# PolarisRisingWar/rgb-experiment

Hardware: AMD Instinct MI355X
Metric: aggregated edges/sec (full-graph GCN d=128, reference epoch = train fwd+bwd+Adam + 2 eval fwd) (higher is better)
Workload: dtype f32

## Files before the change

include/rgbx_hip.h:

```cpp
#ifndef RGBX_HIP_H
#define RGBX_HIP_H

#include <stddef.h>
#include <stdint.h>

#ifdef __cplusplus
extern "C" {
#endif

#define RGBX_VERSION 501

#define RGBX_OK 0
#define RGBX_E_ARG (-1)
#define RGBX_E_RANGE (-2)
#define RGBX_E_ALIGN (-3)
#define RGBX_E_WS (-4)
#define RGBX_E_SHAPE (-5)

typedef void* rgbx_stream_t;

enum {
  RGBX_LOOPS_KEEP = 0,
  RGBX_LOOPS_ADD_REMAINING = 1,
  RGBX_LOOPS_REMOVE_ADD = 2
// ... 137 lines not shown
  int64_t N, K, Nout;
  const rgbx_row_split_t* split;
  const float* w_pos;
  float* z_pos_out;
  const uint8_t* col_sel;
} rgbx_fused_layer_t;

int rgbx_fused_layer_f32(const rgbx_fused_layer_t* layer, rgbx_stream_t stream);

int rgbx_blocked_to_rows_f32(const float* src, int64_t blk_cols, int64_t blk_stride, float* dst, int64_t ldd,
                             int64_t n, int64_t d, const float* bias, rgbx_stream_t stream);

int rgbx_appnp_f32(const int32_t* rowptr, const int32_t* col, const float* w, const float* h,
                   int64_t ldh, float* out, float* tmp, int64_t ldo, int64_t N, int64_t d, int K,
                   float alpha, const rgbx_row_split_t* split, rgbx_stream_t stream);


int rgbx_dagnn_gate_fwd_f32(const float* h0, int64_t ld0, const float* hops, int64_t hop_stride, int64_t ldh,
                            const float* s, const float* b, float* out, int64_t ldo, int64_t N, int64_t d, int K,
                            rgbx_stream_t stream);

int rgbx_dagnn_gate_bwd_workspace_bytes(int64_t d, size_t* bytes);
int rgbx_dagnn_gate_bwd_f32(const float* h0, int64_t ld0, const float* hops, int64_t hop_stride, int64_t ldh,
                            const float* s, const float* b, const float* gout, int64_t ldg, float* d0,
                            int64_t ldd0, float* dk, int64_t d_stride, int64_t ldd, float* g_s, float* g_b,
                            void* ws, size_t ws_bytes, int64_t N, int64_t d, int K, rgbx_stream_t stream);


int rgbx_gru_step_supported(int64_t C);
int rgbx_gru_step_f32(const int32_t* rowptr, const int32_t* col, const float* x, int64_t ldx, const float* wt,
                      const float* wt_root, const float* bias, float* out, int64_t ldo, float* z_out, int64_t ldz,
                      float* pre_out, int64_t ldp, int64_t N, int64_t C, const rgbx_row_split_t* split,
                      rgbx_stream_t stream);

int rgbx_gru_gate_fwd_f32(const float* pre, int64_t ldp, const float* x, int64_t ldx, float* out, int64_t ldo,
                          int64_t N, int64_t C, rgbx_stream_t stream);

int rgbx_gru_gate_bwd_f32(const float* pre, int64_t ldp, const float* x, int64_t ldx, const float* gout, int64_t ldg,
                          float* dpre, int64_t lddp, float* dx, int64_t lddx, int64_t N, int64_t C,
                          rgbx_stream_t stream);


int rgbx_gat_scores_f32(const float* hfeat, int64_t ldh, const float* att_src,
                        const float* att_dst, float* a_src, float* a_dst, int64_t n, int H, int C,
                        rgbx_stream_t stream);

int rgbx_gat_scores_bwd_scratch_floats(int64_t n, int H, int C, int64_t* count);

int rgbx_gat_scores_bwd_f32(const float* hfeat, int64_t ldh, const float* g_a_src, const float* g_a_dst,
                            int64_t n_dst, const float* att_src, const float* att_dst, float* g_hfeat,
                            int64_t ldgh, float* g_att_src, float* g_att_dst, float* scratch,
                            int64_t scratch_floats, int64_t n, int H, int C, rgbx_stream_t stream);

int rgbx_gat_aggregate_fwd_f32(const int32_t* rowptr, const int32_t* col, const float* hfeat,
                               int64_t ldh, const float* a_src, const float* att_src,
                               float* a_dst, const float* att_dst, const float* out_scale, const float* bias,
                               float* out, int64_t ldo, float* m, float* rden, float* out_pos, float* a_pos,
                               int64_t N, int H, int C, float slope, const rgbx_row_split_t* split,
                               rgbx_stream_t stream);

int rgbx_gat_edge_softmax_f32(const int32_t* rowptr, const int32_t* col, const float* a_src, const float* a_dst,
                              float slope, float* alpha, float* alpha_pos, float* m, float* rden, float* a_pos,
                              int64_t N, const rgbx_row_split_t* split, rgbx_stream_t stream);

int rgbx_gat_bwd_dst_f32(const int32_t* rowptr, const int32_t* col, const float* hfeat,
                         int64_t ldh, const float* a_src, const float* a_dst, const float* m,
                         const float* rden, const float* out, int64_t ldo, const float* gout,
                         int64_t ldg, float* nodeq, float* g_a_dst, int64_t N, int H, int C,
                         float slope, rgbx_stream_t stream);

int rgbx_gat_bwd_prep_f32(const float* a_dst, const float* m, const float* rden, const float* out,
                          int64_t ldo, const float* bias, const float* gout, int64_t ldg, float* nodeq,
                          const float* out_pos, const float* a_pos, float slope, float* g_a_dst,
                          int64_t N, int H, int C, rgbx_stream_t stream);

int rgbx_gat_bwd_src_f32(const int32_t* rowptr_t, const int32_t* col_t, const float* hfeat,
                         int64_t ldh, const float* a_src, const float* nodeq, const float* gout,
                         int64_t ldg, float* g_hfeat, int64_t ldgh, float* g_a_src, float* ds,
                         const float* att2, const float* g_a_dst, int64_t N, int H, int C, float slope,
                         const rgbx_row_split_t* split, rgbx_stream_t stream);



int rgbx_supergat_supported(int H, int C);

int rgbx_supergat_loss_records(int64_t N, const rgbx_row_split_t* split, int64_t* count);

int rgbx_supergat_aggregate_fwd_f32(const int32_t* rowptr, const int32_t* col, const float* hfeat, int64_t ldh,
                                    const float* att_l, const float* att_r, const float* bias, float* out, int64_t ldo,
                                    float* m, float* rden, int64_t N, int H, int C, float slope, const uint32_t* seed,
                                    float p_drop, float pos_ratio, float* loss_records, int64_t n_loss_records,
                                    double* pos_stats, const rgbx_row_split_t* split, rgbx_stream_t stream);

int rgbx_supergat_bwd_dst_f32(const int32_t* rowptr, const int32_t* col, const float* hfeat, int64_t ldh,
                              const float* att_l, const float* att_r, const float* m, const float* rden,
                              const float* out, int64_t ldo, const float* bias, const float* gout, int64_t ldg,
                              float* nodeq, float* g_hfeat, int64_t ldgh, float* g_ar, int64_t N, int H, int C,
                              float slope, const uint32_t* seed, float p_drop, float pos_ratio, const float* gl,
                              const rgbx_row_split_t* split, rgbx_stream_t stream);

int rgbx_supergat_bwd_src_f32(const int32_t* rowptr_t, const int32_t* col_t, const int32_t* t2f, const float* hfeat,
                              int64_t ldh, const float* att_l, const float* nodeq, const float* gout, int64_t ldg,
                              float* g_hfeat, int64_t ldgh, float* g_al, int64_t N, int H, int C, float slope,
                              const uint32_t* seed, float p_drop, float pos_ratio, const float* gl,
                              const rgbx_row_split_t* split, rgbx_stream_t stream);

int rgbx_supergat_sample_negatives(const uint64_t* keys, int64_t n_keys, int64_t N, const uint32_t* seed, int64_t n_neg,
                                   int redraws, int64_t* neg, uint8_t* valid, rgbx_stream_t stream);

int rgbx_supergat_neg_loss_fwd_f32(const float* hfeat, int64_t ldh, const int64_t* neg, const uint8_t* valid,
                                   int64_t n_neg, int H, int C, float* loss_records, int64_t n_loss_records,
                                   double* neg_stats, rgbx_stream_t stream);

int rgbx_supergat_neg_loss_bwd_f32(const float* hfeat, int64_t ldh, const int64_t* neg, const uint8_t* valid,
                                   int64_t n_neg, int H, int C, const float* gl, float* g_hfeat, int64_t ldgh,
                                   rgbx_stream_t stream);

int rgbx_supergat_draws_u8(const uint32_t* seed, int64_t nnz, int H, float p_drop, float pos_ratio, uint8_t* pos,
                           uint8_t* drop, rgbx_stream_t stream);



int rgbx_gatv2_supported(int H, int C);

int rgbx_gatv2_fwd_f32(const int32_t* rowptr, const int32_t* col, const float* xl, int64_t ldl, const float* xr,
                       int64_t ldr, const float* att, const float* bias, float* out, int64_t ldo, float* m, float* rden,
                       int64_t N, int H, int C, float slope, const uint32_t* seed, float p_drop,
                       const rgbx_row_split_t* split, rgbx_stream_t stream);

int rgbx_gatv2_att_partial_floats(int64_t N, int H, int C, const rgbx_row_split_t* split, int64_t* count);

int rgbx_gatv2_bwd_dst_f32(const int32_t* rowptr, const int32_t* col, const float* xl, int64_t ldl, const float* xr,
                           int64_t ldr, const float* att, const float* m, const float* rden, const float* out,
                           int64_t ldo, const float* bias, const float* gout, int64_t ldg, float* nodeq, float* g_xr,
                           int64_t ldgr, float* g_att, float* att_partial, int64_t n_att_partial, int64_t N, int H,
                           int C, float slope, const uint32_t* seed, float p_drop, const rgbx_row_split_t* split,
                           rgbx_stream_t stream);

int rgbx_gatv2_bwd_src_f32(const int32_t* rowptr_t, const int32_t* col_t, const int32_t* t2f, const float* xl,
                           int64_t ldl, const float* xr, int64_t ldr, const float* att, const float* nodeq,
                           const float* gout, int64_t ldg, float* g_xl, int64_t ldgl, int64_t N, int H, int C,
                           float slope, const uint32_t* seed, float p_drop, const rgbx_row_split_t* split,
                           rgbx_stream_t stream);

int rgbx_gatv2_draws_u8(const uint32_t* seed, int64_t nnz, int H, float p_drop, uint8_t* keep, rgbx_stream_t stream);


int rgbx_gemm_tn_workspace_bytes(int64_t K, int64_t M, int64_t N, size_t* bytes);

int rgbx_gemm_tn_f32(const float* A, int64_t lda, const float* B, int64_t ldb, float* C, int64_t ldc,
                     float* a_colsum, int64_t K, int64_t M, int64_t N, float alpha, void* workspace,
                     size_t workspace_bytes, rgbx_stream_t stream);


int rgbx_bn_scratch_doubles(int64_t N, int64_t d, int64_t* count);

int rgbx_bn_stats_f32(const float* x, int64_t ldx, int64_t N, int64_t d, double* sums, double* scratch,
                      int64_t scratch_doubles, rgbx_stream_t stream);

int rgbx_bn_finalize_f32(const double* packed, const float* weight, const float* bias, float eps, float momentum,
                         float* running_mean, float* running_var, float* mean, float* rstd, float* scale,
                         float* shift, int64_t d, rgbx_stream_t stream);

int rgbx_fold_bn_linear_f32(const float* W, int64_t ldw, const float* Wr, int64_t ldwr, const float* bias,
                            const float* bias2, const float* gamma, const float* beta, const float* running_mean,
                            const float* running_var, float eps, float* wt, float* wrt, float* b_out, int64_t Nout,
                            int64_t K, rgbx_stream_t stream);

int rgbx_bn_bwd_finalize_f32(const double* glob, const double* local, const double* count, const float* weight,
                             const float* rstd, float* ca, float* cb, float* ck, float* g_weight, float* g_bias,
                             int64_t d, rgbx_stream_t stream);

int rgbx_affine_cols_f32(const float* x, int64_t ldx, const float* scale, const float* shift, float* y,
                         int64_t ldy, int64_t N, int64_t d, rgbx_stream_t stream);

int rgbx_bn_bwd_reduce_f32(const float* gy, int64_t ldg, const float* x, int64_t ldx, const float* mean,
                           const float* rstd, int64_t N, int64_t d, double* sums, double* scratch,
                           int64_t scratch_doubles, rgbx_stream_t stream);

int rgbx_bn_bwd_apply_f32(const float* gy, int64_t ldg, const float* x, int64_t ldx, const float* mean,
                          const float* rstd, const float* ca, const float* cb, const float* ck, float* gx,
                          int64_t ldgx, int64_t N, int64_t d, rgbx_stream_t stream);


int rgbx_masked_nll_scratch_doubles(int64_t N, int want_accuracy, int64_t* count);

int rgbx_masked_nll_fwd_f32(const float* logp, int64_t ld, const int64_t* y, const uint8_t* mask,
                            int64_t N, int64_t C, double* stats, double* scratch,
                            int64_t scratch_doubles, int want_accuracy, rgbx_stream_t stream);

int rgbx_masked_nll_bwd_f32(const int64_t* y, const uint8_t* mask, int64_t N, int64_t C,
                            const float* scale, float* grad, int64_t ldg, rgbx_stream_t stream);

int rgbx_masked_ce_fwd_f32(const float* logits, int64_t ld, const int64_t* y, const uint8_t* mask, int64_t N,
                           int64_t C, double* stats, double* scratch, int64_t scratch_doubles,
                           rgbx_stream_t stream);

int rgbx_masked_ce_fwd_blocked_f32(const float* logits, int64_t blk_cols, int64_t blk_stride, const float* bias,
                                   const int64_t* y, const uint8_t* mask, int64_t N, int64_t C, double* stats,
                                   double* scratch, int64_t scratch_doubles, rgbx_stream_t stream);

int rgbx_masked_ce_bwd_f32(const float* logits, int64_t ld, const int64_t* y, const uint8_t* mask, int64_t N,
                           int64_t C, const float* scale, float* grad, int64_t ldg, rgbx_stream_t stream);


int rgbx_coalesce_workspace_bytes(int64_t E, int64_t N, int mirror, size_t* bytes);
int rgbx_coalesce_keys_i64(const int64_t* row, const int64_t* col, int64_t E, int64_t N, int mirror,
                           uint64_t* keys_out, uint64_t* counts, void* workspace, size_t workspace_bytes,
                           rgbx_stream_t stream);
int rgbx_split_edge_keys_i64(const uint64_t* keys, const uint64_t* counts, int64_t cap, int64_t N, int64_t* out_row,
                             int64_t* out_col, rgbx_stream_t stream);

int rgbx_py_random_shuffle_i64(int64_t seed, int64_t n, int64_t* perm);


int rgbx_gather_rows_f32(const float* src, int64_t lds, const int32_t* idx, int64_t n, int64_t d,
                         float* dst, int64_t ldd, rgbx_stream_t stream);

int rgbx_scatter_add_rows_f32(const float* src, int64_t lds, const int32_t* idx, int64_t n,
                              int64_t d, float* dst, int64_t ldd, rgbx_stream_t stream);

int rgbx_paced_copy_f32(const float* src, float* dst, int64_t n, int workgroups, int nontemporal, rgbx_stream_t stream);



int rgbx_faconv_supported(int64_t C);

int rgbx_faconv_scores_f32(const float* x, int64_t ldx, const float* att_l, const float* att_r, float* alr, int64_t N,
                           int64_t C, rgbx_stream_t stream);

int rgbx_faconv_fwd_f32(const int32_t* rowptr, const int32_t* col, const float* w, const float* x, int64_t ldx,
                        const float* alr, const float* x0, int64_t ldx0, float eps, float* out, int64_t ldo, int64_t N,
                        int64_t C, const uint32_t* seed, float p_drop, const rgbx_row_split_t* split,
                        rgbx_stream_t stream);

int rgbx_faconv_bwd_dst_f32(const int32_t* rowptr, const int32_t* col, const float* w, const float* x, int64_t ldx,
                            const float* alr, const float* gout, int64_t ldg, float* g_alr, int64_t N, int64_t C,
                            const uint32_t* seed, float p_drop, const rgbx_row_split_t* split, rgbx_stream_t stream);

int rgbx_faconv_bwd_src_f32(const int32_t* rowptr_t, const int32_t* col_t, const float* w_t, const int32_t* t2f,
                            const float* x, int64_t ldx, const float* alr, const float* gout, int64_t ldg,
                            const float* att_l, const float* att_r, float* g_alr, float* g_x, int64_t ldgx, int64_t N,
                            int64_t C, const uint32_t* seed, float p_drop, const rgbx_row_split_t* split,
                            rgbx_stream_t stream);

int rgbx_faconv_edge_coef_f32(const int32_t* rowptr, const int32_t* col, const float* w, const int32_t* slot,
                              const float* alr, int transposed, int64_t N, const uint32_t* seed, float p_drop,
                              float* coef, float* q, rgbx_stream_t stream);

int rgbx_faconv_edge_dot_f32(const int32_t* rowptr, const int32_t* col, const float* q, const float* a, int64_t lda,
                             const float* b, int64_t ldb, float* out, int64_t out_stride, int64_t N, int64_t C,
                             rgbx_stream_t stream);

int rgbx_faconv_draws_u8(const uint32_t* seed, int64_t nnz, float p_drop, uint8_t* keep, rgbx_stream_t stream);

#ifdef __cplusplus
}
#endif
#endif
```

rgb_experiment_amd/_lib.py:

```python
import ctypes
import os

import torch

_HERE = os.path.dirname(os.path.abspath(__file__))
LIB_PATH = os.path.join(_HERE, "csrc", "librgbx_hip.so")

_P = ctypes.c_void_p
_I64 = ctypes.c_int64
_I = ctypes.c_int
_F = ctypes.c_float

class RowSplit(ctypes.Structure):
    _fields_ = [("threshold", ctypes.c_int32), ("n_chunks", ctypes.c_int32), ("n_long", ctypes.c_int32),
                ("chunk_begin", ctypes.c_void_p), ("chunk_end", ctypes.c_void_p), ("chunk_row", ctypes.c_void_p),
                ("long_row", ctypes.c_void_p),
                ("long_chunk_ptr", ctypes.c_void_p), ("partial", ctypes.c_void_p)]


class CeEpilogue(ctypes.Structure):
    _fields_ = [("y", ctypes.c_void_p), ("mask", ctypes.c_void_p), ("grad_scale", ctypes.c_void_p),
                ("stats", ctypes.c_void_p), ("scratch", ctypes.c_void_p), ("mask_groups", ctypes.c_int32),
                ("rows", ctypes.c_void_p), ("n_rows", ctypes.c_int64), ("skip_unselected", ctypes.c_int32)]


class SpmmEpilogue(ctypes.Structure):
    _fields_ = [("ce", ctypes.c_void_p), ("n_classes", ctypes.c_int64), ("out_colsums", ctypes.c_void_p),
                ("stats_ws", ctypes.c_void_p), ("stats_ws_bytes", ctypes.c_size_t)]


class FusedLayer(ctypes.Structure):
    _fields_ = [("rowptr", _P), ("col", _P), ("w", _P), ("rs", _P), ("x", _P), ("ldx", _I64),
                ("x_blk_cols", _I64), ("x_blk_stride", _I64), ("wt", _P), ("x_root", _P), ("ldr", _I64),
                ("xr_blk_cols", _I64), ("xr_blk_stride", _I64), ("wt_root", _P), ("bias", _P), ("out", _P),
                ("ldo", _I64), ("out_blk", _P), ("ob_cols", _I64), ("ob_stride", _I64), ("z_out", _P), ("ldz", _I64),
                ("pre_scale", _P), ("pre_shift", _P), ("pre_rowsum", _P), ("out_colsums", _P), ("stats_ws", _P),
                ("stats_ws_bytes", ctypes.c_size_t), ("ce", _P), ("N", _I64), ("K", _I64), ("Nout", _I64),
                ("split", _P), ("w_pos", _P), ("z_pos_out", _P), ("col_sel", _P)]


SIGNATURES = {
    "rgbx_csr_workspace_bytes": [_I64, _I64, ctypes.POINTER(ctypes.c_size_t)],
    "rgbx_csr_build": [_P, _P, _I64, _I64, _I, _P, _P, _P, _P, ctypes.c_size_t, _P],
    "rgbx_deg_inv_sqrt_f32": [_P, _I64, _P, _P],
    "rgbx_gcn_norm_f32": [_P, _P, _I64, _P, _P, _P],
    "rgbx_inv_degree_f32": [_P, _I64, _P, _P],
    "rgbx_loop_weights_f32": [_P, _P, _P, _I64, _I64, _I, _F, _P, _P, _P],
    "rgbx_edge_slot_weights_f32": [_P, _I64, _P, _I64, _P, _P, _P],
    "rgbx_weighted_deg_inv_sqrt_f32": [_P, _P, _I64, _P, _P],
    "rgbx_gcn_norm_weighted_f32": [_P, _P, _P, _I64, _P, _P, _P],
    "rgbx_edge_dot_supported": [_I64],
    "rgbx_edge_dot_f32": [_P, _P, _P, _I64, _P, _I64, _P, _I64, _I64, _P, _P],
    "rgbx_gcn_norm_bwd_f32": [_P, _P, _P, _P, _P, _P, _P, _P, _P, _P, _I64, _I64, _P, _P, _P],
    "rgbx_spmm_csr_f32": [_P, _P, _P, _P, _P, _I64, _P, _I64, _P, _P, _I64, _I64, _I64, _F, _F, _P, _P],
    "rgbx_spmm_csr_extremum_supported": [_I64],
    "rgbx_spmm_csr_extremum_f32": [_P, _P, _P, _I64, _P, _I64, _P, _I64, _I64, _I, _P, _P],
    "rgbx_extremum_bwd_f32": [_P, _P, _P, _P, _I64, _P, _P, _I64, _I64, _I64, _P, _P],
    "rgbx_spmm_csr_epilogue_supported": [_I64],
    "rgbx_spmm_csr_epilogue_f32": [_P, _P, _P, _P, _P, _I64, _P, _I64, _P, _P, _I64, _I64, _I64, _F, _F, _P, _P, _P],
    "rgbx_spmm_csr_short_rows_supported": [_I64],
    "rgbx_spmm_csr_short_rows_f32": [_P, _P, _P, _P, _I64, _P, _P, _I64, _I64, _I64, _P],
    "rgbx_spmm_linear_supported": [_I64, _I64, _I],
    "rgbx_spmm_linear_stats_workspace_bytes": [_I64, _I64, ctypes.POINTER(ctypes.c_size_t)],
    "rgbx_spmm_linear_f32": [_P, _P, _P, _P, _P, _I64, _P, _P, _I64, _P, _P, _P, _I64, _P, _I64, _P, _P, _P, _P, _P,
                             ctypes.c_size_t, _P, _I64, _I64, _I64, _P, _P],
    "rgbx_fused_layer_f32": [_P, _P],
    "rgbx_blocked_to_rows_f32": [_P, _I64, _I64, _P, _I64, _I64, _I64, _P, _P],
    "rgbx_appnp_f32": [_P, _P, _P, _P, _I64, _P, _P, _I64, _I64, _I64, _I, _F, _P, _P],
    "rgbx_dagnn_gate_fwd_f32": [_P, _I64, _P, _I64, _I64, _P, _P, _P, _I64, _I64, _I64, _I, _P],
    "rgbx_dagnn_gate_bwd_workspace_bytes": [_I64, ctypes.POINTER(ctypes.c_size_t)],
    "rgbx_dagnn_gate_bwd_f32": [_P, _I64, _P, _I64, _I64, _P, _P, _P, _I64, _P, _I64, _P, _I64, _I64, _P, _P, _P,
                                ctypes.c_size_t, _I64, _I64, _I, _P],
    "rgbx_gru_step_supported": [_I64],
    "rgbx_gru_step_f32": [_P, _P, _P, _I64, _P, _P, _P, _P, _I64, _P, _I64, _P, _I64, _I64, _I64, _P, _P],
    "rgbx_gru_gate_fwd_f32": [_P, _I64, _P, _I64, _P, _I64, _I64, _I64, _P],
    "rgbx_gru_gate_bwd_f32": [_P, _I64, _P, _I64, _P, _I64, _P, _I64, _P, _I64, _I64, _I64, _P],
    "rgbx_gat_scores_f32": [_P, _I64, _P, _P, _P, _P, _I64, _I, _I, _P],
    "rgbx_gat_scores_bwd_scratch_floats": [_I64, _I, _I, ctypes.POINTER(ctypes.c_int64)],
    "rgbx_gat_scores_bwd_f32": [_P, _I64, _P, _P, _I64, _P, _P, _P, _I64, _P, _P, _P, _I64, _I64, _I, _I, _P],
    "rgbx_gat_aggregate_fwd_f32": [_P, _P, _P, _I64, _P, _P, _P, _P, _P, _P, _P, _I64, _P, _P, _P, _P, _I64, _I, _I, _F, _P,
                                   _P],
    "rgbx_gat_edge_softmax_f32": [_P, _P, _P, _P, _F, _P, _P, _P, _P, _P, _I64, _P, _P],
    "rgbx_gat_bwd_dst_f32": [_P, _P, _P, _I64, _P, _P, _P, _P, _P, _I64, _P, _I64, _P, _P, _I64, _I, _I,
                             _F, _P],
    "rgbx_gat_bwd_prep_f32": [_P, _P, _P, _P, _I64, _P, _P, _I64, _P, _P, _P, _F, _P, _I64, _I, _I, _P],
    "rgbx_gat_bwd_src_f32": [_P, _P, _P, _I64, _P, _P, _P, _I64, _P, _I64, _P, _P, _P, _P, _I64, _I, _I, _F, _P, _P],
    "rgbx_supergat_supported": [_I, _I],
    "rgbx_supergat_loss_records": [_I64, _P, ctypes.POINTER(ctypes.c_int64)],
    "rgbx_supergat_aggregate_fwd_f32": [_P, _P, _P, _I64, _P, _P, _P, _P, _I64, _P, _P, _I64, _I, _I, _F, _P, _F, _F, _P,
                                        _I64, _P, _P, _P],
    "rgbx_supergat_bwd_dst_f32": [_P, _P, _P, _I64, _P, _P, _P, _P, _P, _I64, _P, _P, _I64, _P, _P, _I64, _P, _I64, _I, _I,
                                  _F, _P, _F, _F, _P, _P, _P],
    "rgbx_supergat_bwd_src_f32": [_P, _P, _P, _P, _I64, _P, _P, _P, _I64, _P, _I64, _P, _I64, _I, _I, _F, _P, _F, _F, _P,
                                  _P, _P],
    "rgbx_supergat_sample_negatives": [_P, _I64, _I64, _P, _I64, _I, _P, _P, _P],
    "rgbx_supergat_neg_loss_fwd_f32": [_P, _I64, _P, _P, _I64, _I, _I, _P, _I64, _P, _P],
    "rgbx_supergat_neg_loss_bwd_f32": [_P, _I64, _P, _P, _I64, _I, _I, _P, _P, _I64, _P],
    "rgbx_supergat_draws_u8": [_P, _I64, _I, _F, _F, _P, _P, _P],
    "rgbx_gatv2_supported": [_I, _I],
    "rgbx_gatv2_fwd_f32": [_P, _P, _P, _I64, _P, _I64, _P, _P, _P, _I64, _P, _P, _I64, _I, _I, _F, _P, _F, _P, _P],
    "rgbx_gatv2_att_partial_floats": [_I64, _I, _I, _P, ctypes.POINTER(ctypes.c_int64)],
    "rgbx_gatv2_bwd_dst_f32": [_P, _P, _P, _I64, _P, _I64, _P, _P, _P, _P, _I64, _P, _P, _I64, _P, _P, _I64, _P, _P, _I64,
                               _I64, _I, _I, _F, _P, _F, _P, _P],
    "rgbx_gatv2_bwd_src_f32": [_P, _P, _P, _P, _I64, _P, _I64, _P, _P, _P, _I64, _P, _I64, _I64, _I, _I, _F, _P, _F, _P,
                               _P],
    "rgbx_gatv2_draws_u8": [_P, _I64, _I, _F, _P, _P],
    "rgbx_gemm_tn_workspace_bytes": [_I64, _I64, _I64, ctypes.POINTER(ctypes.c_size_t)],
    "rgbx_gemm_tn_f32": [_P, _I64, _P, _I64, _P, _I64, _P, _I64, _I64, _I64, _F, _P, ctypes.c_size_t, _P],
    "rgbx_bn_scratch_doubles": [_I64, _I64, ctypes.POINTER(ctypes.c_int64)],
    "rgbx_bn_stats_f32": [_P, _I64, _I64, _I64, _P, _P, _I64, _P],
    "rgbx_bn_finalize_f32": [_P, _P, _P, _F, _F, _P, _P, _P, _P, _P, _P, _I64, _P],
    "rgbx_fold_bn_linear_f32": [_P, _I64, _P, _I64, _P, _P, _P, _P, _P, _P, _F, _P, _P, _P, _I64, _I64, _P],
    "rgbx_bn_bwd_finalize_f32": [_P, _P, _P, _P, _P, _P, _P, _P, _P, _P, _I64, _P],
    "rgbx_affine_cols_f32": [_P, _I64, _P, _P, _P, _I64, _I64, _I64, _P],
    "rgbx_bn_bwd_reduce_f32": [_P, _I64, _P, _I64, _P, _P, _I64, _I64, _P, _P, _I64, _P],
    "rgbx_bn_bwd_apply_f32": [_P, _I64, _P, _I64, _P, _P, _P, _P, _P, _P, _I64, _I64, _I64, _P],
    "rgbx_masked_nll_scratch_doubles": [_I64, _I, ctypes.POINTER(ctypes.c_int64)],
    "rgbx_masked_nll_fwd_f32": [_P, _I64, _P, _P, _I64, _I64, _P, _P, _I64, _I, _P],
    "rgbx_masked_ce_fwd_f32": [_P, _I64, _P, _P, _I64, _I64, _P, _P, _I64, _P],
    "rgbx_masked_ce_fwd_blocked_f32": [_P, _I64, _I64, _P, _P, _P, _I64, _I64, _P, _P, _I64, _P],
    "rgbx_masked_ce_bwd_f32": [_P, _I64, _P, _P, _I64, _I64, _P, _P, _I64, _P],
    "rgbx_masked_nll_bwd_f32": [_P, _P, _I64, _I64, _P, _P, _I64, _P],
    "rgbx_coalesce_workspace_bytes": [_I64, _I64, _I, ctypes.POINTER(ctypes.c_size_t)],
    "rgbx_coalesce_keys_i64": [_P, _P, _I64, _I64, _I, _P, _P, _P, ctypes.c_size_t, _P],
    "rgbx_split_edge_keys_i64": [_P, _P, _I64, _I64, _P, _P, _P],
    "rgbx_gather_rows_f32": [_P, _I64, _P, _I64, _I64, _P, _I64, _P],
    "rgbx_scatter_add_rows_f32": [_P, _I64, _P, _I64, _I64, _P, _I64, _P],
    "rgbx_paced_copy_f32": [_P, _P, _I64, _I, _I, _P],
    "rgbx_py_random_shuffle_i64": [_I64, _I64, _P],
    "rgbx_faconv_supported": [_I64],
    "rgbx_faconv_scores_f32": [_P, _I64, _P, _P, _P, _I64, _I64, _P],
    "rgbx_faconv_fwd_f32": [_P, _P, _P, _P, _I64, _P, _P, _I64, _F, _P, _I64, _I64, _I64, _P, _F, _P, _P],
    "rgbx_faconv_bwd_dst_f32": [_P, _P, _P, _P, _I64, _P, _P, _I64, _P, _I64, _I64, _P, _F, _P, _P],
    "rgbx_faconv_bwd_src_f32": [_P, _P, _P, _P, _P, _I64, _P, _P, _I64, _P, _P, _P, _P, _I64, _I64, _I64, _P, _F, _P,
                                _P],
    "rgbx_faconv_edge_coef_f32": [_P, _P, _P, _P, _P, _I, _I64, _P, _F, _P, _P, _P],
    "rgbx_faconv_edge_dot_f32": [_P, _P, _P, _P, _I64, _P, _I64, _P, _I64, _I64, _I64, _P],
    "rgbx_faconv_draws_u8": [_P, _I64, _F, _P, _P],
}
EXPORTS = ["rgbx_version", "rgbx_last_error_string"] + list(SIGNATURES)

_lib = None


def bind(path, strict=True):
    lib = ctypes.CDLL(path)
    lib.rgbx_version.restype = _I
    lib.rgbx_version.argtypes = []
    lib.rgbx_last_error_string.restype = ctypes.c_char_p
    lib.rgbx_last_error_string.argtypes = []
    for name, argtypes in SIGNATURES.items():
        if not strict and not hasattr(lib, name):
            continue
        fn = getattr(lib, name)
        fn.restype = _I
        fn.argtypes = argtypes
    return lib


def load():
    global _lib
    if _lib is not None:
        return _lib
    if not os.path.exists(LIB_PATH):
        raise RuntimeError(
            f"rgb_experiment_amd: {LIB_PATH} is not built — run `python -c 'import __graft_entry__ as g; "
            "g.build()'` (or `make -C rgb_experiment_amd/csrc`). There is no CPU fallback.")
    _lib = bind(LIB_PATH)
    return _lib


def use(lib):
    global _lib
    _lib = lib


def check(rc, what):
    if rc != 0:
        msg = load().rgbx_last_error_string().decode(errors="replace")
        kind = "argument error" if rc < 0 else "hipError"
        raise RuntimeError(f"{what} failed ({kind} {rc}): {msg}")


def require_device(*tensors):
    for t in tensors:
        if t is not None and not t.is_cuda:
            raise RuntimeError(
                "rgb_experiment_amd: the message-passing path runs in HIP kernels on an MI355X device; "
                f"got a tensor on '{t.device}'. There is no CPU fallback (oracle/ is test-only).")


def stream_ptr():
    return torch.cuda.current_stream().cuda_stream


def ptr(t):
    return 0 if t is None else t.data_ptr()


def mat(t, name="tensor"):
    if t.dtype != torch.float32 or t.dim() != 2:
        raise RuntimeError(f"{name}: expected a 2-D float32 tensor, got {t.dtype} {tuple(t.shape)}")
    if t.size(1) > 1 and t.stride(1) != 1:
        raise RuntimeError(f"{name}: rows must be contiguous (stride {t.stride()})")
    ld = t.stride(0) if t.size(0) > 1 else max(t.size(1), 1)
    return t.data_ptr(), ld
```

rgb_experiment_amd/csrc/bn.hip:

```cpp
#include "rgbx_common.h"

namespace rgbx {
namespace {

constexpr int kMaxBlocks = 1024;

struct ColMap {
  int cv;
  int rg;
};

__host__ __device__ inline ColMap col_map(int d, int vec) {
  int cv = (d + vec - 1) / vec;
  if (cv > 256) cv = 256;
  ColMap m{cv, 256 / cv};
  return m;
}

template <int VEC, bool BWD>
__global__ void __launch_bounds__(256)
col_reduce_kernel(const float* __restrict__ a, int64_t lda, const float* __restrict__ b, int64_t ldb,
                  const float* __restrict__ mean, const float* __restrict__ rstd, int64_t N, int d,
                  double* __restrict__ part) {
  extern __shared__ double sh[];
  const ColMap M = col_map(d, VEC);
  const int tid = threadIdx.x;
  const int cvi = tid % M.cv, rgi = tid / M.cv;
  const bool thread_ok = rgi < M.rg;
  const int stride_c = M.cv * VEC;
  for (int cbase = 0; cbase < d; cbase += stride_c) {
    const int c = cbase + cvi * VEC;
    const bool active = thread_ok && c < d;
    double s0[VEC], s1[VEC];
    float mu[VEC], rs[VEC];
#pragma unroll
    for (int i = 0; i < VEC; ++i) { s0[i] = s1[i] = 0.0; mu[i] = 0.f; rs[i] = 1.f; }
    if (BWD && active) {
      load_vec<VEC>(mu, mean + c);
      load_vec<VEC>(rs, rstd + c);
    }
    if (active) {
      for (int64_t r = (int64_t)blockIdx.x * M.rg + rgi; r < N; r += (int64_t)gridDim.x * M.rg) {
        float va[VEC];
        load_vec<VEC>(va, a + r * lda + c);
        if constexpr (BWD) {
          float vb[VEC];
          load_vec<VEC>(vb, b + r * ldb + c);
#pragma unroll
          for (int i = 0; i < VEC; ++i) {
            s0[i] += (double)va[i];
            s1[i] += (double)(va[i] * ((vb[i] - mu[i]) * rs[i]));
          }
        } else {
#pragma unroll
          for (int i = 0; i < VEC; ++i) {
            s0[i] += (double)va[i];
            s1[i] += (double)va[i] * (double)va[i];
          }
        }
      }
    }
    __syncthreads();
    if (thread_ok) {
#pragma unroll
      for (int i = 0; i < VEC; ++i) {
        sh[(rgi * 2 + 0) * stride_c + cvi * VEC + i] = s0[i];
        sh[(rgi * 2 + 1) * stride_c + cvi * VEC + i] = s1[i];
      }
    }
    __syncthreads();
    if (rgi == 0 && active) {
#pragma unroll
      for (int i = 0; i < VEC; ++i) {
        if (c + i < d) {
          double t0 = 0.0, t1 = 0.0;
          for (int g = 0; g < M.rg; ++g) {
            t0 += sh[(g * 2 + 0) * stride_c + cvi * VEC + i];
            t1 += sh[(g * 2 + 1) * stride_c + cvi * VEC + i];
          }
          part[((int64_t)blockIdx.x * 2 + 0) * d + c + i] = t0;
          part[((int64_t)blockIdx.x * 2 + 1) * d + c + i] = t1;
        }
      }
    }
  }
}

__global__ void __launch_bounds__(256)
col_finish_kernel(const double* __restrict__ part, int n_blocks, int d, double* __restrict__ sums) {
  __shared__ double sh[32][8];
  const int j = threadIdx.x & 7, q = threadIdx.x >> 3;
  const int c = blockIdx.x * 8 + j;
  double s = 0.0;
  if (c < 2 * d) {
    const int which = c / d, col = c % d;
    for (int b = q; b < n_blocks; b += 32) s += part[((int64_t)b * 2 + which) * d + col];
  }
  sh[q][j] = s;
  __syncthreads();
  if (q == 0 && c < 2 * d) {
    double t = 0.0;
#pragma unroll
    for (int k = 0; k < 32; ++k) t += sh[k][j];
    sums[c] = t;
  }
}

template <int VEC>
__global__ void __launch_bounds__(256)
affine_kernel(const float* __restrict__ x, int64_t ldx, const float* __restrict__ scale,
              const float* __restrict__ shift, float* __restrict__ y, int64_t ldy, int64_t N, int d) {
  const int per_row = (d + VEC - 1) / VEC;
  const int64_t total = N * per_row;
  for (int64_t idx = (int64_t)blockIdx.x * blockDim.x + threadIdx.x; idx < total;
       idx += (int64_t)gridDim.x * blockDim.x) {
    const int64_t r = idx / per_row;
    const int c = (int)(idx % per_row) * VEC;
    float v[VEC], sc[VEC], sf[VEC];
    load_vec<VEC>(v, x + r * ldx + c);
    load_vec<VEC>(sc, scale + c);
    load_vec<VEC>(sf, shift + c);
#pragma unroll
    for (int i = 0; i < VEC; ++i) v[i] = fmaf(v[i], sc[i], sf[i]);
    store_vec<VEC>(y + r * ldy + c, v);
  }
}

template <int VEC>
__global__ void __launch_bounds__(256)
bn_bwd_apply_kernel(const float* __restrict__ gy, int64_t ldg, const float* __restrict__ x, int64_t ldx,
                    const float* __restrict__ mean, const float* __restrict__ rstd, const float* __restrict__ ca,
                    const float* __restrict__ cb, const float* __restrict__ ck, float* __restrict__ gx,
                    int64_t ldgx, int64_t N, int d) {
  const int per_row = (d + VEC - 1) / VEC;
  const int64_t total = N * per_row;
  for (int64_t idx = (int64_t)blockIdx.x * blockDim.x + threadIdx.x; idx < total;
       idx += (int64_t)gridDim.x * blockDim.x) {
    const int64_t r = idx / per_row;
    const int c = (int)(idx % per_row) * VEC;
    float g[VEC], v[VEC], mu[VEC], rs[VEC], a[VEC], b[VEC], k[VEC];
    load_vec<VEC>(g, gy + r * ldg + c);
    load_vec<VEC>(v, x + r * ldx + c);
    load_vec<VEC>(mu, mean + c);
    load_vec<VEC>(rs, rstd + c);
    load_vec<VEC>(a, ca + c);
    load_vec<VEC>(b, cb + c);
    load_vec<VEC>(k, ck + c);
#pragma unroll
    for (int i = 0; i < VEC; ++i) g[i] = (g[i] - a[i] - (v[i] - mu[i]) * rs[i] * b[i]) * k[i];
    store_vec<VEC>(gx + r * ldgx + c, g);
  }
}

int reduce_grid(int64_t N, int d, int vec) {
  const ColMap M = col_map(d, vec);
  int64_t b = cdiv(N, (int64_t)M.rg * 16);
  if (b > kMaxBlocks) b = kMaxBlocks;
  return (int)(b < 1 ? 1 : b);
}

bool vec4_ok(int64_t d, std::initializer_list<const void*> ptrs, std::initializer_list<int64_t> lds) {
  bool ok = d % 4 == 0;
  for (const void* p : ptrs) ok = ok && aligned16(p);
  for (int64_t ld : lds) ok = ok && ld % 4 == 0;
  return ok;
}

template <bool BWD>
int run_reduce(const float* a, int64_t lda, const float* b, int64_t ldb, const float* mean, const float* rstd,
               int64_t N, int64_t d, double* sums, double* scratch, int64_t scratch_doubles, hipStream_t s,
               const char* name) {
  if (N < 0 || d <= 0 || !sums) return fail(RGBX_E_ARG, "%s: bad argument", name);
  if (d >= INT32_MAX) return fail(RGBX_E_RANGE, "%s: d exceeds int32", name);
  if (N == 0) {
    RGBX_HIP(hipMemsetAsync(sums, 0, 2 * d * sizeof(double), s));
    return RGBX_OK;
  }
  if (!a || lda < d || (BWD && (!b || ldb < d || !mean || !rstd)) || !scratch)
    return fail(RGBX_E_ARG, "%s: null pointer or leading dimension < d", name);
  const bool v4 = BWD ? vec4_ok(d, {a, b, mean, rstd}, {lda, ldb}) : vec4_ok(d, {a}, {lda});
  const int vec = v4 ? 4 : 1;
  const int grid = reduce_grid(N, (int)d, vec);
  if (scratch_doubles < (int64_t)grid * 2 * d)
    return fail(RGBX_E_WS, "%s: scratch %lld < %lld doubles", name, (long long)scratch_doubles,
                (long long)grid * 2 * d);
  const ColMap M = col_map((int)d, vec);
  const size_t lds = (size_t)M.rg * 2 * M.cv * vec * sizeof(double);
  if (v4)
    col_reduce_kernel<4, BWD><<<grid, 256, lds, s>>>(a, lda, b, ldb, mean, rstd, N, (int)d, scratch);
  else
    col_reduce_kernel<1, BWD><<<grid, 256, lds, s>>>(a, lda, b, ldb, mean, rstd, N, (int)d, scratch);
  RGBX_CHECK_LAUNCH(name);
  col_finish_kernel<<<(int)cdiv(2 * d, 8), 256, 0, s>>>(scratch, grid, (int)d, sums);
  RGBX_CHECK_LAUNCH("col_finish_kernel");
  return RGBX_OK;
}

__global__ void __launch_bounds__(256)
bn_finalize_kernel(const double* __restrict__ packed, const float* __restrict__ weight,
                   const float* __restrict__ bias, float eps, float momentum, float* __restrict__ running_mean,
                   float* __restrict__ running_var, float* __restrict__ mean, float* __restrict__ rstd,
                   float* __restrict__ scale, float* __restrict__ shift, int d) {
  const int c = blockIdx.x * blockDim.x + threadIdx.x;
  if (c >= d) return;
  const double n = packed[2 * d];
  const double m64 = packed[c] / n;
  double v64 = packed[d + c] / n - m64 * m64;
  v64 = v64 > 0.0 ? v64 : 0.0;
  const float m = (float)m64, var = (float)v64;
  const float r = 1.0f / sqrtf(var + eps);
  const float sc = weight[c] * r;
  mean[c] = m;
  rstd[c] = r;
  scale[c] = sc;
  shift[c] = bias[c] - m * sc;
  if (running_mean) {
    const double nm1 = n > 1.0 ? n - 1.0 : 1.0;
    const float unbiased = var * (float)(n / nm1);
    running_mean[c] = running_mean[c] * (1.0f - momentum) + momentum * m;
    running_var[c] = running_var[c] * (1.0f - momentum) + momentum * unbiased;
  }
}

__global__ void __launch_bounds__(256)
bn_bwd_finalize_kernel(const double* __restrict__ glob, const double* __restrict__ local,
                       const double* __restrict__ count, const float* __restrict__ weight,
                       const float* __restrict__ rstd, float* __restrict__ ca, float* __restrict__ cb,
                       float* __restrict__ ck, float* __restrict__ g_weight, float* __restrict__ g_bias, int d) {
  const int c = blockIdx.x * blockDim.x + threadIdx.x;
  if (c >= d) return;
  const double n = *count;
  ca[c] = (float)(glob[c] / n);
  cb[c] = (float)(glob[d + c] / n);
  ck[c] = weight[c] * rstd[c];
  g_bias[c] = (float)local[c];
  g_weight[c] = (float)local[d + c];
}

__global__ void __launch_bounds__(256)
fold_bn_linear_kernel(const float* __restrict__ W, int64_t ldw, const float* __restrict__ Wr, int64_t ldwr,
                      const float* __restrict__ bias, const float* __restrict__ bias2,
                      const float* __restrict__ gamma, const float* __restrict__ beta,
                      const float* __restrict__ rmean, const float* __restrict__ rvar, float eps,
                      float* __restrict__ wt, float* __restrict__ wrt, float* __restrict__ b_out, int Nout, int K) {
  __shared__ float tile[2][32][33];
  __shared__ float sc[32];
  const int n0 = blockIdx.x * 32, k0 = blockIdx.y * 32;
  const int tx = threadIdx.x & 31, ty = threadIdx.x >> 5;
  if (threadIdx.x < 32) {
    const int n = n0 + threadIdx.x;
    float s = 1.f, t = 0.f;
    if (n < Nout && gamma) {
      s = gamma[n] * (1.0f / sqrtf(rvar[n] + eps));
      t = beta[n] - rmean[n] * s;
    }
    sc[threadIdx.x] = s;
    if (n < Nout && b_out && blockIdx.y == 0) {
      float b = bias ? bias[n] : 0.f;
      if (bias2) b += bias2[n];
      b_out[n] = b * s + t;
    }
  }
  for (int r = ty; r < 32; r += 8) {
    const int n = n0 + r, k = k0 + tx;
    const bool ok = n < Nout && k < K;
    tile[0][r][tx] = ok ? W[(int64_t)n * ldw + k] : 0.f;
    if (Wr) tile[1][r][tx] = ok ? Wr[(int64_t)n * ldwr + k] : 0.f;
  }
  __syncthreads();
  for (int r = ty; r < 32; r += 8) {
    const int k = k0 + r, n = n0 + tx;
    if (k < K && n < Nout) {
      wt[(int64_t)k * Nout + n] = tile[0][tx][r] * sc[tx];
      if (Wr) wrt[(int64_t)k * Nout + n] = tile[1][tx][r] * sc[tx];
    }
  }
}

int elt_grid(int64_t total) {
  int64_t b = cdiv(total, 256);
  return (int)(b < kMaxGrid ? (b < 1 ? 1 : b) : kMaxGrid);
}

}
}

using namespace rgbx;

extern "C" int rgbx_fold_bn_linear_f32(const float* W, int64_t ldw, const float* Wr, int64_t ldwr, const float* bias,
                                       const float* bias2, const float* gamma, const float* beta,
                                       const float* running_mean, const float* running_var, float eps, float* wt,
                                       float* wrt, float* b_out, int64_t Nout, int64_t K, rgbx_stream_t stream) {
  if (Nout <= 0 || K <= 0) return fail(RGBX_E_ARG, "fold_bn_linear: bad size");
  if (!W || !wt || (Wr && !wrt)) return fail(RGBX_E_ARG, "fold_bn_linear: null pointer");
  const bool bn = gamma || beta || running_mean || running_var;
  if (bn && !(gamma && beta && running_mean && running_var))
    return fail(RGBX_E_ARG, "fold_bn_linear: gamma, beta, running_mean and running_var go together");
  if (ldw < K || (Wr && ldwr < K)) return fail(RGBX_E_ARG, "fold_bn_linear: leading dimension too small");
  if (Nout >= INT32_MAX || K >= INT32_MAX) return fail(RGBX_E_RANGE, "fold_bn_linear: size exceeds int32");
  dim3 grid((unsigned)cdiv(Nout, 32), (unsigned)cdiv(K, 32));
  fold_bn_linear_kernel<<<grid, 256, 0, (hipStream_t)stream>>>(W, ldw, Wr, ldwr, bias, bias2, gamma, beta, running_mean,
                                                            running_var, eps, wt, wrt, b_out, (int)Nout, (int)K);
// ... 80 lines not shown
```

rgb_experiment_amd/csrc/gemm.hip:

```cpp
#include "rgbx_common.h"

namespace rgbx {
namespace {

constexpr int BM = 128, BN = 128, KT = 32;
using f32x16 = __attribute__((ext_vector_type(16))) float;

template <int W>
__device__ __forceinline__ void stage_tile(float* __restrict__ lds, const float* __restrict__ src,
                                           int64_t ld, int64_t k0, int64_t k_end, int c0, int ncols) {
  const int tid = threadIdx.x;
#pragma unroll 4
  for (int p = 0; p < KT * W / 256; ++p) {
    const int idx = p * 256 + tid;
    const int r = idx / W, c = idx % W;
    const int64_t k = k0 + r;
    lds[r * W + c] = (k < k_end && c0 + c < ncols) ? src[k * ld + c0 + c] : 0.f;
  }
}

template <int W>
__device__ __forceinline__ void fetch_tile(float4 (&regs)[KT * (W / 4) / 256], const float* __restrict__ src, int64_t ld,
                                           int64_t k0, int64_t k_end, int c0, int ncols) {
#pragma unroll
  for (int p = 0; p < KT * (W / 4) / 256; ++p) {
    const int idx = p * 256 + threadIdx.x;
    const int r = idx / (W / 4), c = (idx % (W / 4)) * 4;
    const int64_t k = k0 + r;
    regs[p] = make_float4(0.f, 0.f, 0.f, 0.f);
    if (k < k_end && c0 + c < ncols) regs[p] = *reinterpret_cast<const float4*>(src + k * ld + c0 + c);
  }
}

template <int W>
__device__ __forceinline__ void put_tile(float* __restrict__ lds, const float4 (&regs)[KT * (W / 4) / 256]) {
#pragma unroll
  for (int p = 0; p < KT * (W / 4) / 256; ++p) {
    const int idx = p * 256 + threadIdx.x;
    const int r = idx / (W / 4), c = (idx % (W / 4)) * 4;
    *reinterpret_cast<float4*>(lds + r * W + c) = regs[p];
  }
}

template <bool VEC4, int MT>
__global__ void __launch_bounds__(256)
gemm_tn_partial_kernel(const float* __restrict__ A, int64_t lda, const float* __restrict__ B, int64_t ldb,
                       float* __restrict__ part, float* __restrict__ colpart, int64_t K, int M, int N,
                       int64_t slab) {
  constexpr int MI = MT / 64;
  __shared__ float lds[KT * (MT + 128)];
  float* la = lds;
  float* lb = lds + KT * MT;
  const int split = blockIdx.x;
  const int m0 = blockIdx.y * MT, n0 = blockIdx.z * BN;
  const int64_t k_begin = (int64_t)split * slab;
  const int64_t k_end = k_begin + slab < K ? k_begin + slab : K;
  const int wave = threadIdx.x >> 6, lane = threadIdx.x & 63;
  const int wm = (wave >> 1) * (MT / 2), wn = (wave & 1) * 64;
  const int kr = lane >> 5, cc = lane & 31;

  f32x16 acc[MI][2];
#pragma unroll
  for (int i = 0; i < MI; ++i)
#pragma unroll
    for (int j = 0; j < 2; ++j)
#pragma unroll
      for (int r = 0; r < 16; ++r) acc[i][j][r] = 0.f;

  const bool sums = colpart != nullptr && blockIdx.z == 0 && threadIdx.x < MT;
  float csum = 0.f;
  auto consume = [&]() {
    if (sums) {
#pragma unroll 8
      for (int r = 0; r < KT; ++r) csum += la[r * MT + threadIdx.x];
    }
#pragma unroll 4
    for (int kk = 0; kk < KT; kk += 2) {
      float a[MI];
#pragma unroll
      for (int i = 0; i < MI; ++i) a[i] = la[(kk + kr) * MT + wm + i * 32 + cc];
      const float b0 = lb[(kk + kr) * 128 + wn + cc];
      const float b1 = lb[(kk + kr) * 128 + wn + 32 + cc];
#pragma unroll
      for (int i = 0; i < MI; ++i) {
        acc[i][0] = __builtin_amdgcn_mfma_f32_32x32x2f32(a[i], b0, acc[i][0], 0, 0, 0);
        acc[i][1] = __builtin_amdgcn_mfma_f32_32x32x2f32(a[i], b1, acc[i][1], 0, 0, 0);
      }
    }
  };
  if constexpr (VEC4) {
    float4 ra[KT * (MT / 4) / 256], rb[KT * 32 / 256];
    fetch_tile<MT>(ra, A, lda, k_begin, k_end, m0, M);
    fetch_tile<128>(rb, B, ldb, k_begin, k_end, n0, N);
    for (int64_t k0 = k_begin; k0 < k_end; k0 += KT) {
      __syncthreads();
      put_tile<MT>(la, ra);
      put_tile<128>(lb, rb);
      __syncthreads();
      if (k0 + KT < k_end) {
        fetch_tile<MT>(ra, A, lda, k0 + KT, k_end, m0, M);
        fetch_tile<128>(rb, B, ldb, k0 + KT, k_end, n0, N);
      }
      consume();
    }
  } else {
    for (int64_t k0 = k_begin; k0 < k_end; k0 += KT) {
      __syncthreads();
      stage_tile<MT>(la, A, lda, k0, k_end, m0, M);
      stage_tile<128>(lb, B, ldb, k0, k_end, n0, N);
      __syncthreads();
      consume();
    }
  }

  if (sums && m0 + (int)threadIdx.x < M) colpart[(int64_t)split * M + m0 + threadIdx.x] = csum;
  float* out = part + (int64_t)split * M * N;
#pragma unroll
  for (int i = 0; i < MI; ++i)
#pragma unroll
    for (int j = 0; j < 2; ++j)
#pragma unroll
      for (int r = 0; r < 16; ++r) {
        const int m = m0 + wm + i * 32 + (r & 3) + 8 * (r >> 2) + 4 * kr;
        const int n = n0 + wn + j * 32 + cc;
        if (m < M && n < N) out[(int64_t)m * N + n] = acc[i][j][r];
      }
}

__global__ void __launch_bounds__(256)
gemm_tn_reduce_kernel(const float* __restrict__ part, int S, int64_t MN, float* __restrict__ C, int N,
                      int64_t ldc, float alpha) {
  __shared__ float sh[8][32];
  const int j = threadIdx.x & 31, q = threadIdx.x >> 5;
  for (int64_t base = (int64_t)blockIdx.x * 32; base < MN; base += (int64_t)gridDim.x * 32) {
    const int64_t i = base + j;
    float s = 0.f;
    if (i < MN)
      for (int p = q; p < S; p += 8) s += part[(int64_t)p * MN + i];
    __syncthreads();
    sh[q][j] = s;
    __syncthreads();
    if (q == 0 && i < MN) {
      float t = 0.f;
#pragma unroll
      for (int k = 0; k < 8; ++k) t += sh[k][j];
      C[(i / N) * ldc + (i % N)] = alpha * t;
    }
  }
}

int tile_rows(int M) { return M <= 64 ? 64 : BM; }

int choose_splits(int64_t K, int M, int N) {
  const int64_t tiles = cdiv(M, tile_rows(M)) * cdiv(N, BN);
  int64_t s = cdiv(tile_rows(M) == 64 ? 1024 : 768, tiles);
  const int64_t max_s = cdiv(K, 16 * KT);
  if (s > max_s) s = max_s;
  if (s < 1) s = 1;
  return (int)s;
}

}
}

using namespace rgbx;

extern "C" int rgbx_gemm_tn_workspace_bytes(int64_t K, int64_t M, int64_t N, size_t* bytes) {
  if (!bytes || K < 0 || M < 0 || N < 0) return fail(RGBX_E_ARG, "gemm_tn_workspace_bytes: bad argument");
  if (M >= INT32_MAX || N >= INT32_MAX) return fail(RGBX_E_RANGE, "gemm_tn: M or N exceeds int32");
  *bytes = (size_t)choose_splits(K, (int)M, (int)N) * ((size_t)M * (size_t)N + (size_t)M) * sizeof(float);
  return RGBX_OK;
}

extern "C" int rgbx_gemm_tn_f32(const float* A, int64_t lda, const float* B, int64_t ldb, float* C,
                                int64_t ldc, float* a_colsum, int64_t K, int64_t M, int64_t N, float alpha,
                                void* workspace, size_t workspace_bytes, rgbx_stream_t stream) {
  if (K < 0 || M < 0 || N < 0) return fail(RGBX_E_ARG, "gemm_tn: negative size");
  if (M == 0 || N == 0) return RGBX_OK;
  if (!C || (K > 0 && (!A || !B))) return fail(RGBX_E_ARG, "gemm_tn: null pointer");
  if (M >= INT32_MAX || N >= INT32_MAX) return fail(RGBX_E_RANGE, "gemm_tn: M or N exceeds int32");
  if (lda < M || ldb < N || ldc < N) return fail(RGBX_E_ARG, "gemm_tn: leading dimension too small");
  size_t need = 0;
  if (int rc = rgbx_gemm_tn_workspace_bytes(K, M, N, &need)) return rc;
  if (!workspace || workspace_bytes < need)
    return fail(RGBX_E_WS, "gemm_tn: workspace %zu < %zu bytes", workspace_bytes, need);
  hipStream_t s = (hipStream_t)stream;
  const int S = choose_splits(K, (int)M, (int)N);
  const int64_t slab = cdiv(cdiv(K > 0 ? K : 1, S), KT) * KT;
  float* part = static_cast<float*>(workspace);
  float* colpart = a_colsum ? part + (size_t)S * M * N : nullptr;
  const int mt = tile_rows((int)M);
  dim3 grid(S, (unsigned)cdiv(M, mt), (unsigned)cdiv(N, BN));
  const bool v4 = aligned16(A) && aligned16(B) && lda % 4 == 0 && ldb % 4 == 0;
#define RGBX_GEMM_TN(V4, MT) \
  gemm_tn_partial_kernel<V4, MT><<<grid, 256, 0, s>>>(A, lda, B, ldb, part, colpart, K, (int)M, (int)N, slab)
  if (v4) { if (mt == 64) RGBX_GEMM_TN(true, 64); else RGBX_GEMM_TN(true, 128); }
  else { if (mt == 64) RGBX_GEMM_TN(false, 64); else RGBX_GEMM_TN(false, 128); }
#undef RGBX_GEMM_TN
  RGBX_CHECK_LAUNCH("gemm_tn_partial_kernel");
  const int64_t MN = M * N;
  int64_t rb = cdiv(MN, 32);
  if (rb > kMaxGrid) rb = kMaxGrid;
  gemm_tn_reduce_kernel<<<(int)rb, 256, 0, s>>>(part, S, MN, C, (int)N, ldc, alpha);
  RGBX_CHECK_LAUNCH("gemm_tn_reduce_kernel");
  if (a_colsum) {
    gemm_tn_reduce_kernel<<<(int)cdiv(M, 32), 256, 0, s>>>(colpart, S, M, a_colsum, (int)M, M, 1.0f);
    RGBX_CHECK_LAUNCH("gemm_tn_reduce_kernel");
  }
  return RGBX_OK;
}
```

rgb_experiment_amd/csrc/rgbx_common.h:

```cpp
#pragma once
#include <cstring>
#include <hip/hip_runtime.h>

#include <algorithm>
#include <cstdarg>
#include <cstdint>
#include <cstdio>
#include <initializer_list>

#include "../../include/rgbx_hip.h"

namespace rgbx {

constexpr int kWave = 64;

char* err_buf();

inline int fail(int code, const char* fmt, ...) {
  va_list ap;
  va_start(ap, fmt);
  vsnprintf(err_buf(), 256, fmt, ap);
  va_end(ap);
  return code;
}

inline int hip_fail(hipError_t e, const char* what) {
  snprintf(err_buf(), 256, "%s: %s", what, hipGetErrorString(e));
  return (int)e;
}

#define RGBX_CHECK_LAUNCH(what)                               \
  do {                                                        \
    hipError_t e_ = hipGetLastError();                        \
    if (e_ != hipSuccess) return ::rgbx::hip_fail(e_, what);  \
  } while (0)

#define RGBX_HIP(call)                                         \
  do {                                                         \
    hipError_t e_ = (call);                                    \
    if (e_ != hipSuccess) return ::rgbx::hip_fail(e_, #call);  \
  } while (0)

inline bool aligned16(const void* p) { return (reinterpret_cast<uintptr_t>(p) & 15u) == 0; }

inline int64_t cdiv(int64_t a, int64_t b) { return (a + b - 1) / b; }

template <int VEC> struct VecT;
template <> struct VecT<4> { using type = float4; };
template <> struct VecT<2> { using type = float2; };
template <> struct VecT<1> { using type = float; };

template <int VEC>
__device__ __forceinline__ void load_vec(float (&v)[VEC], const float* p) {
  using V = typename VecT<VEC>::type;
  const V t = *reinterpret_cast<const V*>(p);
  if constexpr (VEC == 4) { v[0] = t.x; v[1] = t.y; v[2] = t.z; v[3] = t.w; }
  else if constexpr (VEC == 2) { v[0] = t.x; v[1] = t.y; }
  else { v[0] = t; }
}

template <int VEC>
__device__ __forceinline__ void store_vec(float* p, const float (&v)[VEC]) {
  using V = typename VecT<VEC>::type;
  V t;
  if constexpr (VEC == 4) { t.x = v[0]; t.y = v[1]; t.z = v[2]; t.w = v[3]; }
  else if constexpr (VEC == 2) { t.x = v[0]; t.y = v[1]; }
  else { t = v[0]; }
  *reinterpret_cast<V*>(p) = t;
}

constexpr int kMaxGrid = 256 * 8 * 4;

}
```

rgb_experiment_amd/models/_stack.py:

```python
import torch
import torch.nn as nn
import torch.nn.functional as F

from ..nn import BatchNorm1d


class ModelOutput(dict):

    _LAZY = ("out", "x")

    def __init__(self, logits):
        super().__init__(emb=logits)

    def _log_probs(self):
        out = F.log_softmax(dict.__getitem__(self, "emb"), dim=1)
        dict.__setitem__(self, "out", out)
        dict.__setitem__(self, "x", out)
        return out

    def __missing__(self, key):
        if key in self._LAZY:
            return self._log_probs()
        raise KeyError(key)

    def get(self, key, default=None):
        if key in self._LAZY and not dict.__contains__(self, key):
            return self._log_probs()
        return dict.get(self, key, default)

    def __contains__(self, key):
        return key in self._LAZY or dict.__contains__(self, key)

    def keys(self):
        return ["out", "emb", "x"]

    def __iter__(self):
        return iter(self.keys())

    def __len__(self):
        return 3

    def values(self):
        return [self[k] for k in self.keys()]

    def items(self):
        return [(k, self[k]) for k in self.keys()]

    def copy(self):
        return dict(self.items())

    def pop(self, key, *default):
        if key in self._LAZY and not dict.__contains__(self, key):
            self._log_probs()
        return dict.pop(self, key, *default)

    def __eq__(self, other):
        return dict(self.items()) == other

    __hash__ = None

    def __repr__(self):
        return repr(dict(self.items()))


def model_output(logits):
    return ModelOutput(logits)


class ConvStack(nn.Module):

    def __init__(self, num_layers, dropout_rate, widths, make_conv, bn_width):
        super().__init__()
        if num_layers < 2:
            raise ValueError("num_layers must be at least 2")
        self.num_layers = num_layers
        self.dropout_rate = dropout_rate
        self.convs = nn.ModuleList(make_conv(i, widths[i], widths[i + 1]) for i in range(num_layers))
        self.bns = nn.ModuleList(BatchNorm1d(bn_width) for _ in range(num_layers - 1))

    def forward(self, x, edge_index, edge_weight=None):
        return model_output(self._run(x, edge_index, edge_weight=edge_weight))

    def masked_ce(self, x, edge_index, y, mask, edge_weight=None):
        return self._run(x, edge_index, ce=(y, mask), edge_weight=edge_weight)

    def masked_ce_pair(self, x, edge_index, y, mask_a, mask_b, edge_weight=None):
        return self._run(x, edge_index, ce=(y, (mask_a, mask_b)), edge_weight=edge_weight)[1]

    def _run(self, x, edge_index, ce=None, edge_weight=None):
        from .. import ops
        last = self.num_layers - 1
        ew = {}
        if edge_weight is not None:
            if any(type(c).__name__ != "GCNConv" for c in self.convs):
                raise ValueError(f"{type(self).__name__}: edge_weight is taken by stacks of GCNConv only")
            ew["edge_weight"] = edge_weight
        learned = edge_weight is not None and edge_weight.requires_grad and torch.is_grad_enabled()
        pending = None
        if self.training and torch.is_grad_enabled():
            self._train_forwards = getattr(self, "_train_forwards", 0) + 1
        folded = self._eval_operands() if (not torch.is_grad_enabled() and not self.training and x.is_cuda) else None
        agg0 = (self._input_aggregate(x, edge_index, edge_weight)
                if getattr(self, "cache_input_aggregate", False) and not learned else None)
        if folded is not None and agg0 is None and getattr(self, "collapse_eval", True):
            out = self._run_collapsed(x, edge_index, ce, edge_weight)
            if out is not None:
                return out
        for i, conv in enumerate(self.convs):
            bn = self.bns[i] if i < last else None
            if i == 0 and agg0 is not None and i < last:
                if folded is not None and folded[0] is not None:
                    x = conv.forward_from_aggregate(agg0, x, folded=folded[0])
                    continue
                if torch.is_grad_enabled() or bn is None or bn.training:
                    want = (bn is not None and bn.training and torch.is_grad_enabled()
                            and hasattr(bn, "begin_training_step"))
                    x, pending = conv.forward_from_aggregate(agg0, x, want_colsums=want), bn
                    continue
            if folded is not None and pending is None and folded[i] is not None:
                res = conv.forward_folded(x, edge_index, folded[i], ce=ce if i == last else None, **ew)
                if res is not None:
                    x = res
                    continue
            extra = dict(ew)
            if (bn is not None and bn.training and torch.is_grad_enabled() and getattr(conv, "emits_colsums", False)
                    and hasattr(bn, "begin_training_step")):
                extra["want_colsums"] = True
            if (i == last and ce is not None and getattr(conv, "accepts_ce", False)
                    and (not isinstance(ce[1], (tuple, list)) or getattr(conv, "accepts_ce_pair", False))):
                extra["ce"] = ce
            if pending is not None:
                sums = getattr(x, ops.COLSUMS, None)
                after = getattr(conv, "forward_after_bn", None)
                if after is not None:
                    x, pending = after(x, edge_index, pending, colsums=sums, **extra), bn
                    continue
                x, pending = (pending(x, colsums=sums) if sums is not None else pending(x)), None
            affine = None
            if bn is not None and getattr(conv, "folds_post_affine", False) and not torch.is_grad_enabled():
                fold = getattr(bn, "eval_affine", None)
                affine = fold() if fold is not None else None
            if affine is not None:
                x = conv(x, edge_index, post_affine=affine, **ew)
            else:
                x, pending = conv(x, edge_index, **extra), bn
        if ce is not None and not isinstance(x, tuple):
            x = ops.ce_from_logits(x, ce[0], ce[1])
        return x


def _layer_maps(conv):
    from ..graph import LOOPS_ADD_REMAINING, LOOPS_KEEP, LOOPS_REMOVE_ADD
    name = type(conv).__name__
    if getattr(conv, "aggr", "mean") != "mean":
        return None
    if name == "GCNConv":
        return conv.lin.weight, None, conv.bias, "gcn", LOOPS_ADD_REMAINING
    if name == "MySAGEConv" and conv.add_self_loops:
        return conv.lin_l.weight, conv.lin_r.weight, conv.lin_l.bias + conv.lin_r.bias, "mean", LOOPS_REMOVE_ADD
    if name == "SAGEConv":
        return conv.lin_l.weight, conv.lin_r.weight, conv.lin_l.bias, "mean", LOOPS_KEEP
    return None


def _collapsed_operands(self):
    from .. import ops
    tensors = list(self.parameters()) + list(self.buffers())
    key = (getattr(self, "_train_forwards", 0), ops.weights_epoch()) + tuple((t._version, t.data_ptr()) for t in tensors)
    cached = getattr(self, "_collapsed", None)
    if cached is not None and cached[0] == key:
        return cached[1]
    out = None
    convs, last = list(self.convs), self.num_layers - 1
    maps = [_layer_maps(c) for c in convs]
    C = getattr(convs[-1], "out_channels", 0)
    Cp = (C + 3) // 4 * 4
    if (all(m is not None for m in maps) and len({(m[3], m[4]) for m in maps}) == 1 and 0 < Cp <= 256
            and all(c.out_channels > Cp for c in convs[:-1])):
        affines = [getattr(self.bns[i], "eval_affine", lambda: None)() for i in range(last)]
        if all(a is not None for a in affines):
            with torch.no_grad():
                Q, d = None, None
                for l, (wl, wr, b, _, _) in enumerate(maps):
                    scale, shift = affines[l] if l < last else (None, None)
                    ml = wl.t() if scale is None else wl.t() * scale[None, :]
                    mr = None if wr is None else (wr.t() if scale is None else wr.t() * scale[None, :])
                    if Q is None:
                        Q, d = [mr, ml], [None, None]
                    else:
                        nq, nd = [None] * (len(Q) + 1), [None] * (len(Q) + 1)
                        for k in range(len(Q)):
                            for src, m, dst in ((Q, mr, k), (Q, ml, k + 1)):
                                if src[k] is not None and m is not None:
                                    nq[dst] = src[k] @ m if nq[dst] is None else nq[dst] + src[k] @ m
                            for m, dst in ((mr, k), (ml, k + 1)):
                                if d[k] is not None and m is not None:
                                    nd[dst] = d[k] @ m if nd[dst] is None else nd[dst] + d[k] @ m
                        Q, d = nq, nd
                    const = b if scale is None else b * scale + shift
                    d[0] = const if d[0] is None else d[0] + const
                pad = torch.nn.functional.pad
                have = [k for k, q in enumerate(Q) if q is not None]
                weight = torch.cat([pad(Q[k].t(), (0, 0, 0, Cp - C)) for k in have], dim=0).contiguous()
                shifts = [None if v is None else pad(v.detach(), (0, Cp - C)).contiguous() for v in d]
                out = (weight, have, shifts, C, Cp, maps[0][3], maps[0][4])
    self._collapsed = (key, out)
    return out


def _run_collapsed(self, x, edge_index, ce, edge_weight=None):
    from .. import ops
    from ..graph import get_graph
    operands = self._collapsed_operands()
    if operands is None:
        return None
    weight, have, shifts, C, Cp, kind, loops_mode = operands
    graph = get_graph(edge_index, x.size(0), loops_mode, edge_weight)
    if getattr(graph, "is_distributed", False) or not ops.rows_epilogue_ok(graph, Cp, x, None if ce is None else ce[0]):
        return None
    z = ops.linear(x, weight)
    block = {k: z[:, j * Cp:(j + 1) * Cp] for j, k in enumerate(have)}
    w, rs = ops._kind_weights(graph, kind)
    top = len(shifts) - 1
    u = block[top]
    for k in range(top - 1, 0, -1):
        u = ops.spmm_raw(graph.fwd, w, rs, u, y=block.get(k), a=1.0, b=1.0, bias=shifts[k], kind=f"{kind}_fwd")
    if ce is None:
        return ops.spmm_raw(graph.fwd, w, rs, u, y=block.get(0), a=1.0, b=1.0, bias=shifts[0], kind=f"{kind}_fwd")[:, :C]
    labels, mask = ce
    _, stats = ops.spmm_epilogue_raw(graph.fwd, w, rs, u, y=block.get(0), a=1.0, b=1.0, bias=shifts[0],
                                     ce=(labels, mask, None), n_classes=C, kind=f"{kind}_fwd")
    return None, stats


ConvStack._collapsed_operands = _collapsed_operands
ConvStack._run_collapsed = _run_collapsed


def _eval_operands(self):
    tensors = list(self.parameters()) + list(self.buffers())
    from .. import ops
    key = (getattr(self, "_train_forwards", 0), ops.weights_epoch()) + tuple((t._version, t.data_ptr()) for t in tensors)
    cached = getattr(self, "_folded_eval", None)
    if cached is None or cached[0] != key:
        last = self.num_layers - 1
        out = []
        for i, conv in enumerate(self.convs):
            bn = self.bns[i] if i < last else None
            make = getattr(conv, "eval_operands", None)
            ok = make is not None and (bn is None or (hasattr(bn, "eval_affine") and bn.affine and bn.track_running_stats))
            out.append(make(bn) if ok else None)
        cached = (key, out)
        self._folded_eval = cached
    return cached[1]


ConvStack._eval_operands = _eval_operands


def _input_aggregate(self, x, edge_index, edge_weight=None):
    if x.requires_grad or not x.is_cuda:
        return None
    key = (x.data_ptr(), x._version, tuple(x.shape), edge_index.data_ptr(), edge_index._version, tuple(edge_index.shape))
    if edge_weight is not None:
        key += (edge_weight.data_ptr(), edge_weight._version, tuple(edge_weight.shape))
    cached = getattr(self, "_agg0", None)
    if cached is None or cached[0] != key:
        make = getattr(self.convs[0], "aggregate_input", None)
        args = (x, edge_index) if edge_weight is None else (x, edge_index, edge_weight)
        cached = (key, make(*args) if make is not None else None, x, edge_index, edge_weight)
        self._agg0 = cached
    return cached[1]


ConvStack._input_aggregate = _input_aggregate


def _weighted_call(fn, fwd):
    import inspect
    return set(fwd) == {"x", "edge_index", "edge_weight"} and "edge_weight" in inspect.signature(fn).parameters


def masked_ce_pair(model, fwd, y, mask_a, mask_b):
    from .. import ops
    fn = getattr(model, "masked_ce_pair", None)
    if fn is not None and set(fwd) == {"x", "edge_index"} and fwd["x"].is_cuda:
        return fn(fwd["x"], fwd["edge_index"], y, mask_a, mask_b)
    if fn is not None and fwd["x"].is_cuda and _weighted_call(fn, fwd):
        return fn(fwd["x"], fwd["edge_index"], y, mask_a, mask_b, edge_weight=fwd["edge_weight"])
    emb = model(**fwd)["emb"]
    return torch.stack([ops.masked_ce_accuracy(emb, y, mask_a), ops.masked_ce_accuracy(emb, y, mask_b)])


def masked_ce(model, fwd, y, mask):
    from .. import ops
    fn = getattr(model, "masked_ce", None)
    if fn is not None and set(fwd) == {"x", "edge_index"} and fwd["x"].is_cuda:
        return fn(fwd["x"], fwd["edge_index"], y, mask)
    if fn is not None and fwd["x"].is_cuda and _weighted_call(fn, fwd):
        return fn(fwd["x"], fwd["edge_index"], y, mask, edge_weight=fwd["edge_weight"])
    return ops.ce_from_logits(model(**fwd)["emb"], y, mask)
# ... 1 lines not shown
```

rgb_experiment_amd/nn/batchnorm.py:

```python
import ctypes

import torch
import torch.nn as nn

from .. import _lib


def _scratch(n, d, device):
    cnt = ctypes.c_int64(0)
    _lib.check(_lib.load().rgbx_bn_scratch_doubles(n, d, ctypes.byref(cnt)), "rgbx_bn_scratch_doubles")
    return torch.empty(cnt.value, dtype=torch.float64, device=device), cnt.value


def column_sums(x):
    if not x.is_cuda:
        xd = x.double()
        return torch.stack([xd.sum(0), (xd * xd).sum(0)])
    px, ldx = _lib.mat(x, "x")
    n, d = x.shape
    sums = torch.empty((2, d), dtype=torch.float64, device=x.device)
    scratch, cnt = _scratch(n, d, x.device)
    _lib.check(_lib.load().rgbx_bn_stats_f32(px, ldx, n, d, _lib.ptr(sums), _lib.ptr(scratch), cnt, _lib.stream_ptr()),
               "rgbx_bn_stats_f32")
    return sums


def affine_cols(x, scale, shift):
    if not x.is_cuda:
        return x * scale + shift
    px, ldx = _lib.mat(x, "x")
    y = torch.empty((x.size(0), x.size(1)), dtype=torch.float32, device=x.device)
    _lib.check(_lib.load().rgbx_affine_cols_f32(px, ldx, _lib.ptr(scale), _lib.ptr(shift), _lib.ptr(y), y.stride(0),
                                                x.size(0), x.size(1), _lib.stream_ptr()), "rgbx_affine_cols_f32")
    return y


def bwd_sums(gy, x, mean, rstd):
    if not gy.is_cuda:
        xhat = (x - mean) * rstd
        return torch.stack([gy.double().sum(0), (gy * xhat).double().sum(0)])
    pg, ldg = _lib.mat(gy, "gy")
    px, ldx = _lib.mat(x, "x")
    n, d = x.shape
    sums = torch.empty((2, d), dtype=torch.float64, device=x.device)
    scratch, cnt = _scratch(n, d, x.device)
    _lib.check(_lib.load().rgbx_bn_bwd_reduce_f32(pg, ldg, px, ldx, _lib.ptr(mean), _lib.ptr(rstd), n, d, _lib.ptr(sums),
                                                  _lib.ptr(scratch), cnt, _lib.stream_ptr()), "rgbx_bn_bwd_reduce_f32")
    return sums


def bwd_apply(gy, x, mean, rstd, ca, cb, ck):
    if not gy.is_cuda:
        return (gy - ca - (x - mean) * rstd * cb) * ck
    pg, ldg = _lib.mat(gy, "gy")
    px, ldx = _lib.mat(x, "x")
    gx = torch.empty((x.size(0), x.size(1)), dtype=torch.float32, device=x.device)
    _lib.check(_lib.load().rgbx_bn_bwd_apply_f32(pg, ldg, px, ldx, _lib.ptr(mean), _lib.ptr(rstd), _lib.ptr(ca),
                                                 _lib.ptr(cb), _lib.ptr(ck), _lib.ptr(gx), gx.stride(0), x.size(0),
                                                 x.size(1), _lib.stream_ptr()), "rgbx_bn_bwd_apply_f32")
    return gx


class _BNTrain(torch.autograd.Function):

    @staticmethod
    def forward(ctx, x, weight, bias, eps, reduce, running, colsums=None):
        x = x if x.stride(-1) == 1 else x.contiguous()
        mean, rstd, scale, shift, n = train_statistics(x, weight, bias, eps, reduce, running, colsums)
        y = affine_cols(x, scale.contiguous(), shift.contiguous())
        ctx.save_for_backward(x, weight, mean, rstd, n)
        ctx.reduce = reduce
        return y

    @staticmethod
    def backward(ctx, gy):
        x, weight, mean, rstd, n = ctx.saved_tensors
        gx, gw, gb = train_backward(gy, x, weight, mean, rstd, n, ctx.reduce)
        return gx, gw, gb, None, None, None, None


def pack_statistics(x, colsums=None):
    d = x.size(1)
    count = torch.full((1,), float(x.size(0)), dtype=torch.float64, device=x.device)
    sums = colsums if colsums is not None and tuple(colsums.shape) == (2, d) else column_sums(x)
    return torch.cat([sums.reshape(-1), count])


def train_statistics(x, weight, bias, eps, reduce, running, colsums=None, packed=None):
    d = x.size(1)
    if packed is None:
        packed = reduce(pack_statistics(x, colsums))
    n = packed[2 * d:2 * d + 1]
    if x.is_cuda:
        mean, rstd, scale, shift = (torch.empty(d, dtype=torch.float32, device=x.device) for _ in range(4))
        rm, rv, mom = running if running is not None else (None, None, 0.0)
        _lib.check(_lib.load().rgbx_bn_finalize_f32(
            _lib.ptr(packed), _lib.ptr(weight.detach().contiguous()), _lib.ptr(bias.detach().contiguous()),
            float(eps), float(mom), _lib.ptr(rm), _lib.ptr(rv), _lib.ptr(mean), _lib.ptr(rstd), _lib.ptr(scale),
            _lib.ptr(shift), d, _lib.stream_ptr()), "rgbx_bn_finalize_f32")
    else:
        mean64 = packed[:d] / n
        var64 = (packed[d:2 * d] / n - mean64 * mean64).clamp_(min=0.0)
        mean, var = mean64.float(), var64.float()
        rstd = torch.rsqrt(var + eps)
        scale = weight.detach() * rstd
        shift = bias.detach() - mean * scale
        if running is not None:
            rm, rv, mom = running
            unbiased = var * (n / (n - 1).clamp(min=1)).float()
            rm.mul_(1 - mom).add_(mean, alpha=mom)
            rv.mul_(1 - mom).add_(unbiased, alpha=mom)
    return mean, rstd, scale, shift, n


def train_backward(gy, x, weight, mean, rstd, n, reduce, grads_out=None, sums=None):
    gy = gy if gy.stride(-1) == 1 else gy.contiguous()
    d = x.size(1)
    if sums is None:
        local = bwd_sums(gy, x, mean, rstd)
        glob = reduce(local.reshape(-1).clone())
    else:
        local, glob = sums
    if gy.is_cuda:
        ca, cb, ck = (torch.empty(d, dtype=torch.float32, device=gy.device) for _ in range(3))
        gw, gb = grads_out if grads_out is not None else (torch.empty(d, dtype=torch.float32, device=gy.device)
                                                          for _ in range(2))
        _lib.check(_lib.load().rgbx_bn_bwd_finalize_f32(
            _lib.ptr(glob), _lib.ptr(local), _lib.ptr(n), _lib.ptr(weight.detach().contiguous()), _lib.ptr(rstd),
            _lib.ptr(ca), _lib.ptr(cb), _lib.ptr(ck), _lib.ptr(gw), _lib.ptr(gb), d, _lib.stream_ptr()),
            "rgbx_bn_bwd_finalize_f32")
    else:
        glob = glob.reshape(2, -1)
        ca = (glob[0] / n).float().contiguous()
        cb = (glob[1] / n).float().contiguous()
        ck = (weight * rstd).contiguous()
        gw, gb = local[1].float(), local[0].float()
        if grads_out is not None:
            grads_out[0].copy_(gw)
            grads_out[1].copy_(gb)
            gw, gb = grads_out
    return bwd_apply(gy, x, mean, rstd, ca, cb, ck), gw, gb


class _AffineCols(torch.autograd.Function):

    @staticmethod
    def forward(ctx, x, scale, shift):
        x = x if x.stride(-1) == 1 else x.contiguous()
        ctx.save_for_backward(x, scale)
        return affine_cols(x, scale.detach().contiguous(), shift.detach().contiguous())

    @staticmethod
    def backward(ctx, gy):
        x, scale = ctx.saved_tensors
        gy = gy if gy.stride(-1) == 1 else gy.contiguous()
        gx = g_scale = g_shift = None
        if ctx.needs_input_grad[0]:
            gx = affine_cols(gy, scale.detach().contiguous(), torch.zeros_like(scale))
        if ctx.needs_input_grad[1]:
            g_scale = (gy * x).sum(0)
        if ctx.needs_input_grad[2]:
            g_shift = gy.sum(0)
        return gx, g_scale, g_shift


class BatchNorm1d(nn.BatchNorm1d):

    def _reduce(self, packed):
        return packed

    def _reducer(self, x):
        return self._reduce

    def eval_affine(self):
        if self.training or not self.affine or not self.track_running_stats:
            return None
        scale = self.weight * torch.rsqrt(self.running_var + self.eps)
        return scale, self.bias - self.running_mean * scale

    def forward(self, x, colsums=None):
        if x.dim() != 2 or not self.affine or not self.track_running_stats:
            return super().forward(x)
        if not self.training:
            scale, shift = self.eval_affine()
            if torch.is_grad_enabled() and (x.requires_grad or self.weight.requires_grad or self.bias.requires_grad):
                return _AffineCols.apply(x, scale, shift)
            return affine_cols(x if x.stride(-1) == 1 else x.contiguous(), scale.contiguous(), shift.contiguous())
        return _BNTrain.apply(x, self.weight, self.bias, self.eps, self._reducer(x), self.begin_training_step(), colsums)

    def begin_training_step(self):
        with torch.no_grad():
            self.num_batches_tracked += 1
        if self.momentum is None:
            m = 1.0 / float(self.num_batches_tracked)
        else:
            m = self.momentum
        return self.running_mean, self.running_var, m

    def folds_into_next_layer(self, x):
        return (self.training and self.affine and self.track_running_stats and x.dim() == 2 and x.is_cuda
                and torch.is_grad_enabled())
```

rgb_experiment_amd/nn/conv.py:

```python
import math

import torch
import torch.nn as nn

from .. import _lib, ops
from ..graph import LOOPS_ADD_REMAINING, LOOPS_KEEP, LOOPS_REMOVE_ADD, get_graph


def glorot_(t):
    a = math.sqrt(6.0 / (t.size(-2) + t.size(-1)))
    with torch.no_grad():
        t.uniform_(-a, a)
    return t


def _no_weight_grad(edge_weight, who):
    if edge_weight is not None and edge_weight.requires_grad:
        raise ValueError(f"{who}: edge_weight must not require grad (the gradient in the edge weights is implemented for "
                         "GCNConv only)")


AGGRS = {"mean": "mean", "max": "max", "min": "min", "add": "add", "sum": "add"}


def _set_aggr(conv, aggr):
    if aggr not in AGGRS:
        raise ValueError(f"{type(conv).__name__}: aggr must be one of {sorted(AGGRS)}, got {aggr!r}")
    conv.aggr = AGGRS[aggr]
    if conv.aggr != "mean":
        conv.accepts_ce = conv.accepts_ce_pair = conv.folds_post_affine = conv.emits_colsums = False


def _aggregate(x, graph, aggr):
    if getattr(graph, "is_distributed", False):
        raise NotImplementedError(f"aggr='{aggr}' is not implemented on the partitioned (distributed) route")
    if aggr == "add":
        return ops.propagate_sum(x, graph)
    return ops.propagate_max(x, graph) if aggr == "max" else ops.propagate_min(x, graph)


def _finish_composed(out, post_affine, ce):
    if post_affine is not None:
        out = out * post_affine[0] + post_affine[1]
    return out if ce is None else ops.ce_from_logits(out, ce[0], ce[1])


def _forward_folded(conv, x, edge_index, operands, ce, loops_mode, kind, root, edge_weight=None):
    if operands is None or torch.is_grad_enabled() or not x.is_cuda:
        return None
    graph = get_graph(edge_index, x.size(0), loops_mode, edge_weight)
    if getattr(graph, "is_distributed", False) or not ops.fused_linear_ok(graph, conv.in_channels, conv.out_channels,
                                                                          root=root, x=x):
        return None
    wt, b, wtr = operands
    w = graph.w if kind == "gcn" else None
    rs = graph.inv_deg if kind == "mean" else None
    if ce is not None:
        y, mask = ce
        if not ops.fused_ce_ok(graph, conv.in_channels, conv.out_channels, root, x, y):
            return None
        _, _, stats = ops.fused_layer(x, wt, csr=graph.fwd, w=w, rs=rs, bias=b, x_root=x if root else None,
                                      wt_root=wtr if root else None, ce=(y, mask, None), kind=f"{kind}_linear_fwd",
                                      select_rows=True)
        return None, stats
    out, _, _ = ops.fused_layer(x, wt, csr=graph.fwd, w=w, rs=rs, bias=b, x_root=x if root else None,
                                wt_root=wtr if root else None, kind=f"{kind}_linear_fwd")
    return out


def _aggregate_input(x, edge_index, loops_mode, kind, edge_weight=None):
    if edge_weight is not None and edge_weight.requires_grad:
        return None
    graph = get_graph(edge_index, x.size(0), loops_mode, edge_weight)
    if getattr(graph, "is_distributed", False) or not x.is_cuda or x.requires_grad:
        return None
    with torch.no_grad():
        return ops.propagate_gcn(x, graph) if kind == "gcn" else ops.propagate_mean(x, graph)


def _folded_from_aggregate(z, x, operands, root):
    wt, b, wtr = operands
    out, _, _ = ops.fused_layer(z, wt, bias=b, x_root=x if root else None, wt_root=wtr if root else None,
                                kind="cached_aggregate_linear_fwd")
    return out


class GCNConv(nn.Module):

    folds_post_affine = True
    emits_colsums = True

    def __init__(self, in_channels, out_channels):
        super().__init__()
        self.in_channels, self.out_channels = in_channels, out_channels
        self.lin = nn.Linear(in_channels, out_channels, bias=False)
        self.bias = nn.Parameter(torch.zeros(out_channels))
        self.reset_parameters()

    def reset_parameters(self):
        glorot_(self.lin.weight)
        nn.init.zeros_(self.bias)

    accepts_ce = True
    accepts_ce_pair = True

    def forward(self, x, edge_index, edge_weight=None, post_affine=None, want_colsums=False, ce=None):
        if ce is not None:
            return self._ce(x, edge_index, ce, None, None, edge_weight)
        weight, bias = self.lin.weight, self.bias
        if post_affine is not None:
            scale, shift = post_affine
            weight, bias = weight * scale[:, None], bias * scale + shift
        return self._conv(x, edge_index, weight, bias, want_colsums, edge_weight)

    def eval_operands(self, bn=None):
        return ops.fold_bn_linear(self.lin.weight, self.bias, bn=bn)

    def aggregate_input(self, x, edge_index, edge_weight=None):
        if self.in_channels > self.out_channels or not ops.aggregate_linear_ok(self.in_channels, self.out_channels):
            return None
        return _aggregate_input(x, edge_index, LOOPS_ADD_REMAINING, "gcn", edge_weight)

    def forward_from_aggregate(self, z, x, want_colsums=False, folded=None):
        if folded is not None:
            return _folded_from_aggregate(z, x, folded, False)
        return ops.aggregate_linear(z, self.lin.weight, self.bias, want_colsums=want_colsums)

    def forward_folded(self, x, edge_index, operands, ce=None, edge_weight=None):
        return _forward_folded(self, x, edge_index, operands, ce, LOOPS_ADD_REMAINING, "gcn", False, edge_weight)

    @staticmethod
    def _learned(edge_weight):
        return edge_weight is not None and edge_weight.requires_grad and torch.is_grad_enabled()

    def _ce(self, x, edge_index, ce, bn, colsums, edge_weight=None):
        y, mask = ce
        if self._learned(edge_weight):
            if bn is not None:
                x = bn(x, colsums=colsums)
            return ops.ce_from_logits(self.forward(x, edge_index, edge_weight), y, mask)
        graph = get_graph(edge_index, x.size(0), LOOPS_ADD_REMAINING, edge_weight)
        hand_over = bn is not None and bn.folds_into_next_layer(x)
        if ops.fused_ce_ok(graph, self.in_channels, self.out_channels, False, x, y) and (bn is None or hand_over):
            return ops.propagate_linear_ce(x, graph, "gcn", self.lin.weight, self.bias, None, y, mask, bn=bn,
                                           colsums=colsums)
        if bn is not None:
            x = bn(x, colsums=colsums)
        weight, bias, n = ops.pad_rows4(self.lin.weight, self.bias)
        if ops.rows_epilogue_ok(graph, n, x, y) and not ops.fused_linear_ok(graph, self.in_channels, self.out_channels, x=x):
            return ops.propagate_rows_ce(ops.linear(x, weight), graph, "gcn", n, self.out_channels, y, mask, bias=bias)
        return ops.ce_from_logits(self.forward(x, edge_index, edge_weight), y, mask)

    def forward_after_bn(self, x, edge_index, bn, colsums=None, want_colsums=False, ce=None, edge_weight=None):
        if ce is not None:
            return self._ce(x, edge_index, ce, bn, colsums, edge_weight)
        if self._learned(edge_weight):
            return self.forward(bn(x, colsums=colsums), edge_index, edge_weight, want_colsums=want_colsums)
        graph = get_graph(edge_index, x.size(0), LOOPS_ADD_REMAINING, edge_weight)
        if (bn.folds_into_next_layer(x) and not getattr(graph, "is_distributed", False)
                and ops.fused_linear_ok(graph, self.in_channels, self.out_channels, x=x)):
            return ops.bn_propagate_linear(x, bn, graph, "gcn", self.lin.weight, self.bias, colsums=colsums,
                                           want_colsums=want_colsums)
        return self.forward(bn(x, colsums=colsums), edge_index, edge_weight, want_colsums=want_colsums)

    def _conv(self, x, edge_index, weight, bias, want_colsums=False, edge_weight=None):
        graph = get_graph(edge_index, x.size(0), LOOPS_ADD_REMAINING, edge_weight)
        if self._learned(edge_weight):
            return ops.propagate_gcn_edge_weight(ops.linear(x, weight), edge_weight, graph, bias=bias)
        if ops.fused_linear_ok(graph, self.in_channels, self.out_channels, x=x):
            return ops.propagate_linear(x, graph, "gcn", weight, bias, want_colsums=want_colsums)
        if not x.requires_grad and self.in_channels <= self.out_channels:
            return ops.linear(ops.propagate_gcn(x, graph), weight, bias)
        if want_colsums and ops.rows_epilogue_ok(graph, self.out_channels, x):
            return ops.propagate_rows(ops.linear(x, weight), graph, "gcn", bias=bias, want_colsums=True)
        return ops.propagate_gcn(ops.linear(x, weight), graph, bias=bias)


class SAGEConv(nn.Module):

    folds_post_affine = True
    emits_colsums = True

    def __init__(self, in_channels, out_channels, aggr="mean"):
        super().__init__()
        self.in_channels, self.out_channels = in_channels, out_channels
        _set_aggr(self, aggr)
        self.lin_l = nn.Linear(in_channels, out_channels, bias=True)
        self.lin_r = nn.Linear(in_channels, out_channels, bias=False)

    accepts_ce = True
    accepts_ce_pair = True

    def eval_operands(self, bn=None):
        if self.aggr != "mean":
            return None
        return ops.fold_bn_linear(self.lin_l.weight, self.lin_l.bias, root_weight=self.lin_r.weight, bn=bn)

    def aggregate_input(self, x, edge_index):
        if (self.aggr != "mean" or self.in_channels > self.out_channels
                or not ops.aggregate_linear_ok(self.in_channels, self.out_channels, True)):
            return None
        return _aggregate_input(x, edge_index, LOOPS_KEEP, "mean")

    def _forward_composed(self, x, edge_index):
        graph = get_graph(edge_index, x.size(0), LOOPS_KEEP)
        agg = _aggregate(x, graph, self.aggr)
        return ops.linear(agg, self.lin_l.weight, self.lin_l.bias) + ops.linear(x, self.lin_r.weight)

    def forward_from_aggregate(self, z, x, want_colsums=False, folded=None):
        if folded is not None:
            return _folded_from_aggregate(z, x, folded, True)
        return ops.aggregate_linear(z, self.lin_l.weight, self.lin_l.bias, self.lin_r.weight, x, want_colsums)

    def forward_folded(self, x, edge_index, operands, ce=None):
        if self.aggr != "mean":
            return None
        return _forward_folded(self, x, edge_index, operands, ce, LOOPS_KEEP, "mean", True)

    def _ce(self, x, edge_index, ce, bn, colsums):
        y, mask = ce
        graph = get_graph(edge_index, x.size(0), LOOPS_KEEP)
        hand_over = bn is not None and bn.folds_into_next_layer(x)
        if ops.fused_ce_ok(graph, self.in_channels, self.out_channels, True, x, y) and (bn is None or hand_over):
            return ops.propagate_linear_ce(x, graph, "mean", self.lin_l.weight, self.lin_l.bias, self.lin_r.weight, y,
                                           mask, bn=bn, colsums=colsums)
        if bn is not None:
            x = bn(x, colsums=colsums)
        if (ops.rows_epilogue_ok(graph, (self.out_channels + 3) // 4 * 4, x, y)
                and not ops.fused_linear_ok(graph, self.in_channels, self.out_channels, root=True, x=x)):
            h, n = self._transform_first(x, self.lin_l.weight, self.lin_l.bias, self.lin_r.weight)
            return ops.propagate_rows_ce(h, graph, "mean", n, self.out_channels, y, mask)
        return ops.ce_from_logits(self.forward(x, edge_index), y, mask)

    @staticmethod
    def _transform_first(x, w_l, b_l, w_r):
        w_l, b_l, n = ops.pad_rows4(w_l, b_l)
        w_r = ops.pad_rows4(w_r)[0]
        return ops.linear(x, torch.cat([w_l, w_r]), torch.cat([torch.zeros_like(b_l), b_l])), n

    def forward_after_bn(self, x, edge_index, bn, colsums=None, want_colsums=False, ce=None):
        if self.aggr != "mean":
            return _finish_composed(self._forward_composed(bn(x, colsums=colsums), edge_index), None, ce)
        if ce is not None:
            return self._ce(x, edge_index, ce, bn, colsums)
        graph = get_graph(edge_index, x.size(0), LOOPS_KEEP)
        if (bn.folds_into_next_layer(x) and not getattr(graph, "is_distributed", False)
                and ops.fused_linear_ok(graph, self.in_channels, self.out_channels, root=True, x=x)):
            return ops.bn_propagate_linear(x, bn, graph, "mean", self.lin_l.weight, self.lin_l.bias,
                                           root_weight=self.lin_r.weight, colsums=colsums, want_colsums=want_colsums)
        return self.forward(bn(x, colsums=colsums), edge_index, want_colsums=want_colsums)

    def forward(self, x, edge_index, post_affine=None, want_colsums=False, ce=None):
        if self.aggr != "mean":
            return _finish_composed(self._forward_composed(x, edge_index), post_affine, ce)
        if ce is not None:
            return self._ce(x, edge_index, ce, None, None)
        w_l, b_l, w_r = self.lin_l.weight, self.lin_l.bias, self.lin_r.weight
        if post_affine is not None:
            scale, shift = post_affine
            w_l, b_l, w_r = w_l * scale[:, None], b_l * scale + shift, w_r * scale[:, None]
        graph = get_graph(edge_index, x.size(0), LOOPS_KEEP)
        if ops.fused_linear_ok(graph, self.in_channels, self.out_channels, root=True, x=x):
            return ops.propagate_linear(x, graph, "mean", w_l, b_l, root_weight=w_r, want_colsums=want_colsums)
        if self.in_channels > self.out_channels and x.is_cuda and not getattr(graph, "is_distributed", False):
            h, n = self._transform_first(x, w_l, b_l, w_r)
            out = ops.propagate_rows(h, graph, "mean", n=n, want_colsums=want_colsums and n == self.out_channels)
            return out if n == self.out_channels else out[:, :self.out_channels]
        x_r = ops.linear(ops.target_rows(x, graph), w_r)
        if ops.fused_linear_ok(graph, self.in_channels, self.out_channels, x=x):
            return ops.propagate_linear(x, graph, "mean", w_l, b_l) + x_r
        if self.in_channels > self.out_channels:
            return ops.propagate_mean(ops.linear(x, w_l), graph) + b_l + x_r
        agg = ops.propagate_mean(x, graph)
        return ops.linear(agg, w_l, b_l) + x_r


class MySAGEConv(nn.Module):

    folds_post_affine = True
    emits_colsums = True

    def __init__(self, in_channels, out_channels, add_self_loops=True, aggr="mean"):
        super().__init__()
        self.in_channels, self.out_channels = in_channels, out_channels
        self.add_self_loops = add_self_loops
        _set_aggr(self, aggr)
        self.lin_l = nn.Linear(in_channels, out_channels)
        self.lin_r = nn.Linear(in_channels, out_channels)

    accepts_ce = True
    accepts_ce_pair = True

    def _forward_composed(self, x, edge_index):
        graph = get_graph(edge_index, x.size(0), LOOPS_REMOVE_ADD if self.add_self_loops else LOOPS_KEEP)
        h, n = self._transform_both(x, self.lin_l.weight, self.lin_l.bias, self.lin_r.weight, self.lin_r.bias)
        out = _aggregate(h[:, :n], graph, self.aggr) + h[:, n:]
        return out if n == self.out_channels else out[:, :self.out_channels]

    def eval_operands(self, bn=None):
        if not self.add_self_loops or self.aggr != "mean":
            return None
        return ops.fold_bn_linear(self.lin_l.weight, self.lin_l.bias, self.lin_r.bias, root_weight=self.lin_r.weight,
                                  bn=bn)

    def aggregate_input(self, x, edge_index):
        if (not self.add_self_loops or self.aggr != "mean" or self.in_channels > self.out_channels
                or not ops.aggregate_linear_ok(self.in_channels, self.out_channels, True)):
            return None
        return _aggregate_input(x, edge_index, LOOPS_REMOVE_ADD, "mean")

    def forward_from_aggregate(self, z, x, want_colsums=False, folded=None):
        if folded is not None:
            return _folded_from_aggregate(z, x, folded, True)
        return ops.aggregate_linear(z, self.lin_l.weight, self.lin_l.bias + self.lin_r.bias, self.lin_r.weight, x,
                                    want_colsums)

    def forward_folded(self, x, edge_index, operands, ce=None):
        if self.aggr != "mean":
            return None
        return _forward_folded(self, x, edge_index, operands, ce, LOOPS_REMOVE_ADD, "mean", True)

    def _ce(self, x, edge_index, ce, bn, colsums):
        y, mask = ce
# ... 425 lines not shown
```

rgb_experiment_amd/ops.py:

```python
import ctypes

import torch

from . import _lib

_EVENT_SINK = None


def set_event_sink(sink):
    global _EVENT_SINK
    _EVENT_SINK = sink


class Kind(str):
    variant = None


class _Timed:
    def __init__(self, kind, variant=None):
        if variant is not None and _EVENT_SINK is not None:
            kind = Kind(kind)
            kind.variant = variant
        self.kind = kind

# ... 597 lines not shown
                                 _lib.ptr(ce_scratch), groups)
        if select_rows and not dense and w_pos is None:
            if grad_scale is not None:
                ce_arg.skip_unselected = 1
            elif not want_z and z is None and mask is not None:
                rows = selected_rows(y, mask, n_out)
                if rows is not None:
                    ce_arg.rows, ce_arg.n_rows = rows.data_ptr(), rows.numel()
                    keep.append(rows)
        keep += [y, mask, ce_scratch, ce_arg]
        L.ce = ctypes.addressof(ce_arg)
        want_out = grad_scale is not None
    if out is not None:
        if tuple(out.shape) != (N, n_out) or out.stride(1) != 1 or out.dtype != torch.float32:
            raise RuntimeError(f"fused_layer: out is {tuple(out.shape)}, expected a float32 [{N}, {n_out}] with contiguous rows")
    elif want_out:
        out = torch.empty((N, n_out), dtype=torch.float32, device=x.device)
    if out is not None:
        L.out, L.ldo = out.data_ptr(), out.stride(0) if N > 1 else n_out
    else:
        L.ldo = n_out
    if out_blocked is not None:
        L.out_blk, L.ob_cols, L.ob_stride = _blocked(out_blocked, "out_blocked")
        if out_blocked.size(1) != N or out_blocked.size(0) * out_blocked.size(2) != n_out:
            raise RuntimeError(f"fused_layer: out_blocked is {tuple(out_blocked.shape)} for a [{N}, {n_out}] output")
    if z is not None:
        if tuple(z.shape) != (N, K) or z.stride(1) != 1 or z.dtype != torch.float32:
            raise RuntimeError(f"fused_layer: z is {tuple(z.shape)}, expected a float32 [{N}, {K}] with contiguous rows")
    elif want_z or w_pos is not None:
        z = torch.empty((N, K), dtype=torch.float32, device=x.device)
    L.ldz = K
    if z is not None:
        L.z_out, L.ldz = z.data_ptr(), z.stride(0) if N > 1 else K
    z_pos = None
    if w_pos is not None:
        _lib.require_device(w_pos)
        z_pos = torch.empty_strided((N, K), (L.ldz, 1), dtype=torch.float32, device=x.device)
        keep.append(w_pos)
        L.w_pos, L.z_pos_out = w_pos.data_ptr(), z_pos.data_ptr()
    colsums = None
    if want_colsums:
        nbytes = ctypes.c_size_t(0)
        _lib.check(lib.rgbx_spmm_linear_stats_workspace_bytes(N, n_out, ctypes.byref(nbytes)),
                   "rgbx_spmm_linear_stats_workspace_bytes")
        ws = torch.empty(max(nbytes.value, 8), dtype=torch.uint8, device=x.device)
        colsums = torch.empty((2, n_out), dtype=torch.float64, device=x.device)
        keep.append(ws)
        L.out_colsums, L.stats_ws, L.stats_ws_bytes = colsums.data_ptr(), ws.data_ptr(), nbytes.value
    L.N, L.K, L.Nout = N, K, n_out
    variant = None
    if _EVENT_SINK is not None:
        variant = "+".join([name for name, on in (
            ("dense", dense), ("pre", pre is not None), ("root", wt_root is not None), ("z", z is not None),
            ("zpos", w_pos is not None), ("stats", want_colsums), ("ce_stats", ce is not None and ce[2] is None),
            ("ce_grad", ce is not None and ce[2] is not None), ("noout", out is None and out_blocked is None and ce is None),
            ("blk", out_blocked is not None)) if on]) or "plain"
    with _Timed(kind, variant):
        _lib.check(lib.rgbx_fused_layer_f32(ctypes.byref(L), _lib.stream_ptr()), "rgbx_fused_layer_f32")
    del keep
    if groups == 2:
        ce_stats = ce_stats.view(2, 3)
    return out, (z if w_pos is None else (z, z_pos)), (ce_stats if ce is not None else colsums)


def blocked_to_rows(src, out=None, bias=None):
    _lib.require_device(src, bias)
    ptr, bc, bs = _blocked(src, "src")
    n, d = src.size(1), src.size(0) * src.size(2)
    if out is None:
        out = torch.empty((n, d), dtype=torch.float32, device=src.device)
    b = None if bias is None else bias.detach().contiguous()
    _lib.check(_lib.load().rgbx_blocked_to_rows_f32(ptr, bc, bs, out.data_ptr(), out.stride(0), n, d, _lib.ptr(b),
                                                    _lib.stream_ptr()), "rgbx_blocked_to_rows_f32")
    return out


def spmm_linear_raw(csr, w, rs, x, wt, bias=None, want_z=False, x_root=None, wt_root=None, kind="linear", pre=None,
                    want_colsums=False, ce=None, select_rows=False):
    out, z, extra = fused_layer(x, wt, csr=csr, w=w, rs=rs, bias=bias, x_root=x_root if wt_root is not None else None,
                                wt_root=wt_root, pre=pre, want_z=want_z, want_colsums=want_colsums, ce=ce, kind=kind,
                                select_rows=select_rows)
    if ce is not None or want_colsums:
        return out, z, extra
    return out, z


class _AggregateLinear(torch.autograd.Function):

    @staticmethod
    def forward(ctx, z, weight, bias, root_weight, x_root, want_colsums):
        out, _, cs = fused_layer(z, weight_t(weight), bias=None if bias is None else bias.detach(),
                                 x_root=x_root if root_weight is not None else None,
                                 wt_root=None if root_weight is None else weight_t(root_weight),
                                 want_colsums=want_colsums, kind="cached_aggregate_linear_fwd")
        ctx.save_for_backward(z, x_root if root_weight is not None else None)
        ctx.has_bias = bias is not None
        if want_colsums:
            ctx.mark_non_differentiable(cs)
            return out, cs
        return out

    @staticmethod
    def backward(ctx, gy, _g_cs=None):
        z, x_root = ctx.saved_tensors
        gy = gy.contiguous()
        gw = gb = gwr = None
        want_b = ctx.has_bias and ctx.needs_input_grad[2]
        if ctx.needs_input_grad[1]:
            if want_b:
                gw, gb = gemm_tn(gy, z, colsum=True)
            else:
                gw = gemm_tn(gy, z)
        elif want_b:
            gb = gy.sum(0)
        if x_root is not None and ctx.needs_input_grad[3]:
            gwr = gemm_tn(gy, x_root)
        return None, gw, gb, gwr, None, None


def aggregate_linear_ok(in_channels, out_channels, root=False):
    return bool(_lib.load().rgbx_spmm_linear_supported(in_channels, out_channels, int(root)))


def aggregate_linear(z, weight, bias=None, root_weight=None, x_root=None, want_colsums=False):
    return _tag_colsums(_AggregateLinear.apply(z, weight, bias, root_weight, x_root, want_colsums), want_colsums)


def fold_bn_linear(weight, bias=None, bias2=None, root_weight=None, bn=None):
    _lib.require_device(weight, bias, bias2, root_weight)
    W = weight.detach()
    W = W if W.stride(-1) == 1 else W.contiguous()
    n_out, K = W.shape
    Wr = None
    if root_weight is not None:
        Wr = root_weight.detach()
        Wr = Wr if Wr.stride(-1) == 1 else Wr.contiguous()
    wt = torch.empty((K, n_out), dtype=torch.float32, device=W.device)
    wrt = torch.empty_like(wt) if Wr is not None else None
    has_b = bias is not None or bias2 is not None or bn is not None
    b_out = torch.empty(n_out, dtype=torch.float32, device=W.device) if has_b else None
    c = lambda t: None if t is None else t.detach().contiguous()
    b1, b2 = c(bias), c(bias2)
    g = be = rm = rv = None
    eps = 0.0
    if bn is not None:
        g, be, rm, rv, eps = c(bn.weight), c(bn.bias), c(bn.running_mean), c(bn.running_var), bn.eps
    _lib.check(_lib.load().rgbx_fold_bn_linear_f32(
        _lib.ptr(W), W.stride(0), _lib.ptr(Wr), 0 if Wr is None else Wr.stride(0), _lib.ptr(b1), _lib.ptr(b2),
        _lib.ptr(g), _lib.ptr(be), _lib.ptr(rm), _lib.ptr(rv), float(eps), _lib.ptr(wt), _lib.ptr(wrt), _lib.ptr(b_out),
        n_out, K, _lib.stream_ptr()), "rgbx_fold_bn_linear_f32")
    return wt, b_out, wrt


class _PropagateLinear(torch.autograd.Function):

    @staticmethod
    def forward(ctx, x, graph, kind, weight, bias, need_z=True, root_weight=None, x_root=None, want_colsums=False):
        x = x.contiguous()
        xr = x if x_root is None else x_root.contiguous()
        w = graph.w if kind == "gcn" else None
        rs = graph.inv_deg if kind == "mean" else None
        if kind not in ("gcn", "mean", "sum"):
            raise ValueError(kind)
        res = spmm_linear_raw(graph.fwd, w, rs, x, weight_t(weight), None if bias is None else bias.detach(),
                              need_z, xr if root_weight is not None else None,
                              None if root_weight is None else weight_t(root_weight),
                              kind=f"{getattr(graph, 'event_prefix', '')}{kind}_linear_fwd", want_colsums=want_colsums)
        out, z = res[0], res[1]
        ctx.save_for_backward(z, weight, root_weight, xr if root_weight is not None else None)
        ctx.graph, ctx.kind, ctx.has_bias = graph, kind, bias is not None
        if want_colsums:
            ctx.mark_non_differentiable(res[2])
            return out, res[2]
        return out

    @staticmethod
    def backward(ctx, gy, _g_colsums=None):
        z, weight, root_weight, x = ctx.saved_tensors
        g, kind = ctx.graph, ctx.kind
        gy = gy.contiguous()
        gx = gw = gb = gwr = None
        want_b = ctx.has_bias and ctx.needs_input_grad[4]
        if ctx.needs_input_grad[3]:
            if want_b:
                gw, gb = gemm_tn(gy, z, colsum=True)
            else:
                gw = gemm_tn(gy, z)
        elif want_b:
            gb = gy.sum(0)
        if root_weight is not None and ctx.needs_input_grad[6]:
            gwr = gemm_tn(gy, x)
        if ctx.needs_input_grad[0]:
            gx = _propagate_linear_input_grad(g, kind, gy, weight, root_weight)
        return gx, None, None, gw, gb, None, gwr, None, None


def _propagate_linear_input_grad(g, kind, gy, weight, root_weight, ce_sel=None):
    csr = g.bwd
    wt = {"gcn": lambda: g.w_t, "mean": lambda: g.w_mean_t, "sum": lambda: None}[kind]()
    prefix = getattr(g, "event_prefix", "")
    n_out, n_in = weight.shape
    if n_out <= n_in and _lib.load().rgbx_spmm_linear_supported(n_out, n_in, int(root_weight is not None)):
        gx, _, _ = fused_layer(gy, weight.detach().contiguous(), csr=csr, w=wt,
                               x_root=gy if root_weight is not None else None,
                               wt_root=None if root_weight is None else root_weight.detach().contiguous(),
                               col_sel=None if ce_sel is None else selected_cols(*ce_sel), kind=f"{prefix}{kind}_linear_bwd")
        return gx
    gz = gy @ weight
    gr = gy @ root_weight if root_weight is not None else None
    if gr is None:
        return spmm_raw(csr, wt, None, gz, kind=f"{prefix}{kind}_bwd")
    return spmm_raw(csr, wt, None, gz, y=gr, a=1.0, b=1.0, out=gr, kind=f"{prefix}{kind}_bwd")


class _BNPropagateLinear(torch.autograd.Function):

    @staticmethod
    def forward(ctx, x, bn_weight, bn_bias, graph, kind, weight, bias, root_weight, eps, reduce, running, need_z,
                colsums=None, want_colsums=False):
        from .nn import batchnorm as B
        x = x.contiguous()
        mean, rstd, scale, shift, n = B.train_statistics(x, bn_weight, bn_bias, eps, reduce, running, colsums)
        w, rs = (graph.w, None) if kind == "gcn" else (None, graph.inv_deg)
        res = spmm_linear_raw(graph.fwd, w, rs, x, weight_t(weight), None if bias is None else bias.detach(), need_z,
                              x if root_weight is not None else None,
                              None if root_weight is None else weight_t(root_weight), kind=f"{kind}_linear_fwd",
                              pre=(scale, shift, graph.rowsum(kind)), want_colsums=want_colsums)
        out, z = res[0], res[1]
        ctx.save_for_backward(x, bn_weight, mean, rstd, n, z, weight, root_weight, scale, shift)
        ctx.graph, ctx.kind, ctx.has_bias, ctx.reduce = graph, kind, bias is not None, reduce
        if want_colsums:
            ctx.mark_non_differentiable(res[2])
            return out, res[2]
        return out

    @staticmethod
    def backward(ctx, gy, _g_colsums=None):
        from .nn import batchnorm as B
        x, bn_weight, mean, rstd, n, z, weight, root_weight, scale, shift = ctx.saved_tensors
        g, kind = ctx.graph, ctx.kind
        gy = gy.contiguous()
        gw = gb = gwr = None
        if ctx.needs_input_grad[5]:
            gw, gcol = gemm_tn(gy, z, colsum=True)
            gb = gcol if ctx.has_bias and ctx.needs_input_grad[6] else None
        else:
            gcol = gy.sum(0)
            gb = gcol if ctx.has_bias and ctx.needs_input_grad[6] else None
        if root_weight is not None and ctx.needs_input_grad[7]:
            gwr = gemm_tn(gy, x) * scale + gcol[:, None] * shift
        g_h = _propagate_linear_input_grad(g, kind, gy, weight, root_weight)
        gx, g_bnw, g_bnb = B.train_backward(g_h, x, bn_weight, mean, rstd, n, ctx.reduce)
        return gx, g_bnw, g_bnb, None, None, gw, gb, gwr, None, None, None, None, None, None


_SCALE_CACHE = {}


def mask_scale(y, mask, C):
    key = (y.data_ptr(), y._version, y.numel(), None if mask is None else (mask.data_ptr(), mask._version), int(C))
    hit = _SCALE_CACHE.get(key)
    if hit is None:
        sel = (y >= 0) & (y < C)
        if mask is not None:
            sel = sel & mask.bool()
        hit = (_MadeOn((1.0 / sel.sum().double()).float().reshape(1)), y, mask)
        _SCALE_CACHE[key] = hit
        while len(_SCALE_CACHE) > 32:
            _SCALE_CACHE.pop(next(iter(_SCALE_CACHE)))
    return hit[0].get()


_GROUP_MASKS = {}


def group_masks(mask_a, mask_b):
    _lib.require_device(mask_a, mask_b)
    key = (mask_a.data_ptr(), mask_a._version, mask_b.data_ptr(), mask_b._version, mask_a.numel())
    hit = _GROUP_MASKS.get(key)
    if hit is None:
        g = (mask_a.bool().to(torch.uint8) | (mask_b.bool().to(torch.uint8) << 1)).contiguous()
        hit = (_MadeOn(g), mask_a, mask_b)
        _GROUP_MASKS[key] = hit
        while len(_GROUP_MASKS) > 16:
            _GROUP_MASKS.pop(next(iter(_GROUP_MASKS)))
    return hit[0].get()


def ce_selection(y, mask, C):
    sel = (y >= 0) & (y < C)
    if mask is not None:
        sel = sel & mask.bool()
    return sel


def _sel_key(y, mask, C):
    return (y.data_ptr(), y._version, y.numel(),
            None if mask is None else (mask.data_ptr(), mask._version, mask.numel()), int(C))


_SEL_ROWS = {}


def selected_rows(y, mask, C):
    key = _sel_key(y, mask, C)
    hit = _SEL_ROWS.get(key)
    if hit is None:
        if torch.cuda.is_current_stream_capturing():
            return None
        rows = ce_selection(y, mask, C).nonzero().reshape(-1).to(torch.int32).contiguous()
        hit = (_MadeOn(rows), y, mask)
        _SEL_ROWS[key] = hit
        while len(_SEL_ROWS) > 16:
            _SEL_ROWS.pop(next(iter(_SEL_ROWS)))
    return hit[0].get()


_SEL_COLS = {}


def selected_cols(y, mask, C):
    key = _sel_key(y, mask, C)
    hit = _SEL_COLS.get(key)
    if hit is None:
        if torch.cuda.is_current_stream_capturing():
            return None
        hit = (_MadeOn(ce_selection(y, mask, C).to(torch.uint8).contiguous()), y, mask)
        _SEL_COLS[key] = hit
        while len(_SEL_COLS) > 16:
            _SEL_COLS.pop(next(iter(_SEL_COLS)))
    return hit[0].get()



def ce_from_logits(logits, y, mask):
    if isinstance(mask, (tuple, list)):
        return None, torch.stack([masked_ce_accuracy(logits, y, m) for m in mask])
    if torch.is_grad_enabled() and logits.requires_grad:
        return masked_ce_loss(logits, y, mask, with_stats=True)
    stats = masked_ce_accuracy(logits, y, mask)
    return (stats[0] / stats[1]).float(), stats


def fused_ce_ok(graph, in_channels, out_channels, root, x, y):
    return (not _is_dist(graph) and out_channels <= 128 and y is not None and y.is_cuda and y.dtype == torch.int64
            and fused_linear_ok(graph, in_channels, out_channels, root=root, x=x))


class _PropagateLinearCE(torch.autograd.Function):

    @staticmethod
    def forward(ctx, x, graph, kind, weight, bias, root_weight, y, mask, want_grad, bn_weight, bn_bias, bn_args):
        from .nn import batchnorm as B
        x = x.contiguous()
        pre = None
        if bn_weight is not None:
            eps, reduce, running, colsums = bn_args
            mean, rstd, scale, shift, n = B.train_statistics(x, bn_weight, bn_bias, eps, reduce, running, colsums)
            pre = (scale, shift, graph.rowsum(kind))
        w, rs = (graph.w, None) if kind == "gcn" else (None, graph.inv_deg)
        grad_scale = mask_scale(y, mask, weight.size(0)) if want_grad else None
        dlogits, z, stats = spmm_linear_raw(
            graph.fwd, w, rs, x, weight_t(weight), None if bias is None else bias.detach(),
            want_grad and weight.requires_grad, x if root_weight is not None else None,
            None if root_weight is None else weight_t(root_weight), kind=f"{kind}_linear_fwd", pre=pre,
            ce=(y, mask, grad_scale), select_rows=True)
        ctx.graph, ctx.kind, ctx.has_bias, ctx.has_bn = graph, kind, bias is not None, bn_weight is not None
        ctx.ce_sel = (y, mask, weight.size(0)) if want_grad else None
        if want_grad:
            if ctx.has_bn:
                ctx.save_for_backward(dlogits, z, weight, root_weight, x, bn_weight, mean, rstd, n, scale, shift)
                ctx.reduce = bn_args[1]
            else:
                ctx.save_for_backward(dlogits, z, weight, root_weight, x if root_weight is not None else None)
        ctx.mark_non_differentiable(stats)
        if stats.dim() == 2:
            return stats.new_zeros(()).float(), stats
        return (stats[0] / stats[1]).float(), stats

    @staticmethod
    def backward(ctx, g, _g_stats):
        from .nn import batchnorm as B
        saved = ctx.saved_tensors
        if ctx.has_bn:
            gy, z, weight, root_weight, x, bn_weight, mean, rstd, n, scale, shift = saved
        else:
            gy, z, weight, root_weight, x = saved
        graph, kind = ctx.graph, ctx.kind
        g = g.reshape(()).float()
        gw = gb = gwr = gx = g_bnw = g_bnb = None
        gcol = None
        if ctx.needs_input_grad[3]:
            gw, gcol = gemm_tn(gy, z, colsum=True)
        if ctx.has_bias and ctx.needs_input_grad[4]:
            gb = gcol if gcol is not None else gy.sum(0)
        if root_weight is not None and ctx.needs_input_grad[5]:
            if ctx.has_bn:
                gcol = gcol if gcol is not None else gy.sum(0)
                gwr = gemm_tn(gy, x) * scale + gcol[:, None] * shift
            else:
                gwr = gemm_tn(gy, x)
        need_h = ctx.needs_input_grad[0] or (ctx.has_bn and (ctx.needs_input_grad[9] or ctx.needs_input_grad[10]))
        items = [(k, t) for k, t in (("gw", gw), ("gb", gb), ("gwr", gwr)) if t is not None]
        if need_h:
            items.append(("w", weight.detach()))
            if root_weight is not None:
                items.append(("wr", root_weight.detach()))
        sc = dict(zip((k for k, _ in items), torch._foreach_mul([t for _, t in items], g))) if items else {}
        gw, gb, gwr = sc.get("gw"), sc.get("gb"), sc.get("gwr")
        if need_h:
            g_h = _propagate_linear_input_grad(graph, kind, gy, sc["w"], sc.get("wr"), ce_sel=ctx.ce_sel)
            if ctx.has_bn:
                gx, g_bnw, g_bnb = B.train_backward(g_h, x, bn_weight, mean, rstd, n, ctx.reduce)
            else:
                gx = g_h
        return gx, None, None, gw, gb, gwr, None, None, None, g_bnw, g_bnb, None


def propagate_linear_ce(x, graph, kind, weight, bias, root_weight, y, mask, bn=None, colsums=None):
    want_grad = not isinstance(mask, (tuple, list)) and torch.is_grad_enabled() and any(
        t is not None and t.requires_grad
        for t in (weight, x, bias, root_weight) + ((bn.weight, bn.bias) if bn is not None else ()))
    if bn is not None:
        bn_args = (bn.eps, bn._reduce, bn.begin_training_step(), colsums)
        return _PropagateLinearCE.apply(x, graph, kind, weight, bias, root_weight, y, mask, want_grad, bn.weight, bn.bias,
                                        bn_args)
    return _PropagateLinearCE.apply(x, graph, kind, weight, bias, root_weight, y, mask, want_grad, None, None, None)


def bn_propagate_linear(x, bn, graph, kind, weight, bias=None, root_weight=None, colsums=None, want_colsums=False):
    need_z = weight.requires_grad
    return _tag_colsums(_BNPropagateLinear.apply(x, bn.weight, bn.bias, graph, kind, weight, bias, root_weight, bn.eps,
                                                 bn._reduce, bn.begin_training_step(), need_z, colsums, want_colsums),
                        want_colsums)


COLSUMS = "_rgbx_colsums"


def _tag_colsums(res, want_colsums):
    if not want_colsums:
        return res
    out, colsums = res
    setattr(out, COLSUMS, colsums)
    return out


def propagate_linear(x, graph, kind, weight, bias=None, root_weight=None, want_colsums=False):
    if _is_dist(graph):
        return graph.propagate_linear(x, kind, weight, bias, root_weight)
    need_z = torch.is_grad_enabled() and weight.requires_grad
    return _tag_colsums(_PropagateLinear.apply(x, graph, kind, weight, bias, need_z, root_weight, None, want_colsums),
                        want_colsums)


def appnp_raw(csr, w, h, K, alpha, kind="appnp"):
    _lib.require_device(h)
    h = h.contiguous()
    ph, ldh = _lib.mat(h, "h")
    out = torch.empty_like(h)
    tmp = torch.empty_like(h) if K > 1 else None
    po, ldo = _lib.mat(out, "out")
    split, _scratch = csr.split_arg(h.size(1), h.device)
    with _Timed(kind):
        _lib.check(
            _lib.load().rgbx_appnp_f32(_lib.ptr(csr.rowptr), _lib.ptr(csr.col), _lib.ptr(w), ph, ldh, po,
                                       _lib.ptr(tmp), ldo, csr.N, h.size(1), int(K), float(alpha),
                                       None if split is None else ctypes.byref(split), _lib.stream_ptr()),
            "rgbx_appnp_f32")
    return out


class _APPNP(torch.autograd.Function):

    @staticmethod
    def forward(ctx, h, graph, K, alpha):
        ctx.graph, ctx.K, ctx.alpha = graph, K, alpha
        return appnp_raw(graph.fwd, graph.w, h, K, alpha, kind="appnp_fwd")

    @staticmethod
    def backward(ctx, gy):
        g = ctx.graph
        return appnp_raw(g.bwd, g.w_t, gy, ctx.K, ctx.alpha, kind="appnp_bwd"), None, None, None


class _APPNPCE(torch.autograd.Function):

    @staticmethod
    def forward(ctx, h, graph, K, alpha, labels, mask, n_classes, want_grad):
        h = h.contiguous()
        z = appnp_raw(graph.fwd, graph.w, h, K - 1, alpha, kind="appnp_fwd") if K > 1 else h
        grad_scale = mask_scale(labels, mask, n_classes) if want_grad else None
        dlogits, stats = spmm_epilogue_raw(graph.fwd, graph.w, None, z, y=h, a=1.0 - alpha, b=alpha,
                                           ce=(labels, mask, grad_scale), n_classes=n_classes, kind="appnp_fwd")
        ctx.graph, ctx.K, ctx.alpha = graph, K, alpha
        if want_grad:
            ctx.save_for_backward(dlogits)
        ctx.mark_non_differentiable(stats)
        if stats.dim() == 2:
            return stats.new_zeros(()).float(), stats
        return (stats[0] / stats[1]).float(), stats

    @staticmethod
    def backward(ctx, g, _g_stats=None):
        if not ctx.saved_tensors:
            raise RuntimeError("appnp_propagate_ce: backward asked of a forward that was run without want_grad")
        gy = ctx.saved_tensors[0] * g.reshape(()).float()
        gr = ctx.graph
        return appnp_raw(gr.bwd, gr.w_t, gy, ctx.K, ctx.alpha, kind="appnp_bwd"), None, None, None, None, None, None, None


def appnp_propagate_ce(h, graph, K, alpha, n_classes, y, mask):
    pair = isinstance(mask, (tuple, list))
    want_grad = (not pair) and torch.is_grad_enabled() and h.requires_grad
    loss, stats = _APPNPCE.apply(h, graph, int(K), float(alpha), y, mask, int(n_classes), want_grad)
    return (None if pair else loss), stats


def appnp_propagate(h, graph, K, alpha):
    if _is_dist(graph):
        out = graph.appnp(h, K, alpha)
        if out is not None:
            return out
        z = h
        for _ in range(K):
            z = (1.0 - alpha) * graph.propagate(z, "gcn") + alpha * h
        return z
    hp, d = _pad4(h)
    out = _APPNP.apply(hp, graph, K, alpha)
    return out if hp is h else out[:, :d]


class _DAGNNProp(torch.autograd.Function):

    @staticmethod
    def forward(ctx, x, graph, K, s, b):
        lib = _lib.load()
        N, d = x.shape
        x = x.contiguous()
        hops = torch.empty((K, N, d), dtype=torch.float32, device=x.device)
        src = x
        for k in range(K):
            spmm_raw(graph.fwd, graph.w, None, src, out=hops[k], kind="gcn_fwd")
            src = hops[k]
        out = torch.empty_like(x)
        sv = s.detach().reshape(-1).contiguous()
        bv = None if b is None else b.detach().reshape(-1).contiguous()
        with _Timed("dagnn_gate_fwd"):
            _lib.check(lib.rgbx_dagnn_gate_fwd_f32(_lib.ptr(x), x.stride(0), _lib.ptr(hops), N * d, d, _lib.ptr(sv),
                                                   _lib.ptr(bv), _lib.ptr(out), out.stride(0), N, d, K,
                                                   _lib.stream_ptr()), "rgbx_dagnn_gate_fwd_f32")
        ctx.graph, ctx.K, ctx.has_b = graph, K, b is not None
        ctx.save_for_backward(x, hops, sv, bv)
        return out

    @staticmethod
    def backward(ctx, gout):
        lib = _lib.load()
        x, hops, sv, bv = ctx.saved_tensors
        g, K = ctx.graph, ctx.K
        N, d = x.shape
        gout = gout.contiguous()
        d0 = torch.empty_like(x)
        dk = torch.empty((K, N, d), dtype=torch.float32, device=x.device)
        g_s = torch.empty(d, dtype=torch.float32, device=x.device)
        g_b = torch.empty(1, dtype=torch.float32, device=x.device) if ctx.has_b else None
        need = ctypes.c_size_t(0)
        _lib.check(lib.rgbx_dagnn_gate_bwd_workspace_bytes(d, ctypes.byref(need)), "rgbx_dagnn_gate_bwd_workspace_bytes")
        ws = torch.empty(need.value, dtype=torch.uint8, device=x.device)
        with _Timed("dagnn_gate_bwd"):
            _lib.check(lib.rgbx_dagnn_gate_bwd_f32(_lib.ptr(x), x.stride(0), _lib.ptr(hops), N * d, d, _lib.ptr(sv),
                                                   _lib.ptr(bv), _lib.ptr(gout), gout.stride(0), _lib.ptr(d0),
                                                   d0.stride(0), _lib.ptr(dk), N * d, d, _lib.ptr(g_s), _lib.ptr(g_b),
                                                   _lib.ptr(ws), need.value, N, d, K, _lib.stream_ptr()),
                       "rgbx_dagnn_gate_bwd_f32")
        gx = None
        if ctx.needs_input_grad[0]:
            cur = dk[K - 1] if K else d0
            for k in range(K - 1, -1, -1):
                dst = dk[k - 1] if k else d0
                spmm_raw(g.bwd, g.w_t, None, cur, y=dst, a=1.0, b=1.0, out=dst, kind="gcn_bwd")
                cur = dst
            gx = d0
        return gx, None, None, g_s, g_b


def dagnn_prop(x, graph, K, proj_weight, proj_bias=None):
    if _is_dist(graph) or x.size(1) > 256:
        return None
    _lib.require_device(x, proj_weight, proj_bias)
    xp, d = _pad4(x)
    s = proj_weight.reshape(-1)
    if xp is not x:
        s = torch.nn.functional.pad(s, (0, xp.size(1) - d))
    out = _DAGNNProp.apply(xp, graph, int(K), s, proj_bias)
    return out if xp is x else out[:, :d]



GRU_FORMS = ("fused", "composed", "general")
GRU_FORM = None


def gru_step_supported(C):
    return bool(_lib.load().rgbx_gru_step_supported(int(C)))
# ... 780 lines not shown
    if record.get("seed") is None:
        keep = torch.ones(nnz, dtype=torch.uint8, device=dev)
    else:
        keep = torch.empty(nnz, dtype=torch.uint8, device=dev)
        _lib.check(_lib.load().rgbx_faconv_draws_u8(_lib.ptr(record["seed"]), nnz, float(record["p_drop"]), _lib.ptr(keep),
                                                    _lib.stream_ptr()), "rgbx_faconv_draws_u8")
    deg = (csr.rowptr[1:] - csr.rowptr[:-1]).long()
    return {"keep": keep.bool(), "src": csr.col[:nnz].long(),
            "dst": torch.repeat_interleave(torch.arange(csr.N, device=dev), deg)}


def _faconv_edge_coef(csr, w, slot, alr, transposed, seed, p_drop, want_q):
    coef = torch.empty(max(csr.nnz, 1), dtype=torch.float32, device=alr.device)
    q = torch.empty_like(coef) if want_q else None
    with _Timed("faconv_edge_coef"):
        _lib.check(_lib.load().rgbx_faconv_edge_coef_f32(_lib.ptr(csr.rowptr), _lib.ptr(csr.col), _lib.ptr(w),
                                                         _lib.ptr(slot), _lib.ptr(alr), int(transposed), csr.N,
                                                         _lib.ptr(seed), float(p_drop), _lib.ptr(coef), _lib.ptr(q),
                                                         _lib.stream_ptr()), "rgbx_faconv_edge_coef_f32")
    return coef, q


def _faconv_edge_dot(csr, q, a, b, out, column):
    pa, lda = _lib.mat(a, "a")
    pb, ldb = _lib.mat(b, "b")
    with _Timed("faconv_edge_dot"):
        _lib.check(_lib.load().rgbx_faconv_edge_dot_f32(_lib.ptr(csr.rowptr), _lib.ptr(csr.col), _lib.ptr(q), pa, lda, pb,
                                                        ldb, out.data_ptr() + 4 * column, 2, csr.N, a.size(1),
                                                        _lib.stream_ptr()), "rgbx_faconv_edge_dot_f32")


class _FAConv(torch.autograd.Function):

    @staticmethod
    def forward(ctx, x, x0, att_l, att_r, graph, eps, train, p_drop, form, record):
        _lib.require_device(x, x0, att_l, att_r)
        lib = _lib.load()
        csr, N, dev = graph.fwd, graph.fwd.N, x.device
        x = x.contiguous()
        C = x.size(1)
        if x.size(0) != N:
            raise RuntimeError(f"faconv: {x.size(0)} feature rows for a graph of {N} nodes")
        use_x0 = x0 is not None and eps != 0.0
        x0c = x0.contiguous() if use_x0 else None
        att = torch.cat([att_l.detach().reshape(1, C), att_r.detach().reshape(1, C)]).contiguous()
        seed = None
        if train and p_drop > 0.0:
            seed = torch.randint(0, 2 ** 31 - 1, (2,), dtype=torch.int32, device=dev)
        if record is not None:
            record.update(seed=seed, p_drop=float(p_drop))
        alr = torch.empty((N, 2), dtype=torch.float32, device=dev)
        px, ldx = _lib.mat(x, "x")
        with _Timed("faconv_scores"):
            _lib.check(lib.rgbx_faconv_scores_f32(px, ldx, att[0].data_ptr(), att[1].data_ptr(), _lib.ptr(alr), N, C,
                                                  _lib.stream_ptr()), "rgbx_faconv_scores_f32")
        if form == "fused":
            out = torch.empty((N, C), dtype=torch.float32, device=dev)
            po, ldo = _lib.mat(out, "out")
            p0, ld0 = _lib.mat(x0c, "x_0") if use_x0 else (None, 0)
            split, _scratch = csr.split_arg(C + 1, dev)
            with _Timed("faconv_fwd"):
                _lib.check(lib.rgbx_faconv_fwd_f32(_lib.ptr(csr.rowptr), _lib.ptr(csr.col), _lib.ptr(graph.w), px, ldx,
                                                   _lib.ptr(alr), p0, ld0, float(eps), po, ldo, N, C, _lib.ptr(seed),
                                                   float(p_drop), None if split is None else ctypes.byref(split),
                                                   _lib.stream_ptr()), "rgbx_faconv_fwd_f32")
        else:
            coef, _ = _faconv_edge_coef(csr, graph.w, None, alr, 0, seed, p_drop, False)
            out = spmm_raw(csr, coef, None, x, y=x0c, a=1.0, b=float(eps), kind="faconv_fwd_composed")
        ctx.graph, ctx.eps, ctx.p_drop, ctx.form, ctx.use_x0 = graph, float(eps), float(p_drop), form, use_x0
        ctx.att_shapes = (att_l.shape, att_r.shape)
        ctx.save_for_backward(x, alr, att, seed)
        return out

    @staticmethod
    def backward(ctx, gout):
        x, alr, att, seed = ctx.saved_tensors
        g, p_drop = ctx.graph, ctx.p_drop
        lib = _lib.load()
        N, C, dev = x.size(0), x.size(1), x.device
        gout = gout.contiguous()
        g_alr = torch.empty((N, 2), dtype=torch.float32, device=dev)
        px, ldx = _lib.mat(x, "x")
        pg, ldg = _lib.mat(gout, "gout")
        t2f = g.t2f if seed is not None else None
        if ctx.form == "fused":
            g_x = torch.empty_like(x)
            pgx, ldgx = _lib.mat(g_x, "g_x")
            split, _scratch = g.fwd.split_arg(C + 1, dev)
            with _Timed("faconv_bwd_dst"):
                _lib.check(lib.rgbx_faconv_bwd_dst_f32(_lib.ptr(g.fwd.rowptr), _lib.ptr(g.fwd.col), _lib.ptr(g.w), px, ldx,
                                                       _lib.ptr(alr), pg, ldg, _lib.ptr(g_alr), N, C, _lib.ptr(seed), p_drop,
                                                       None if split is None else ctypes.byref(split),
                                                       _lib.stream_ptr()), "rgbx_faconv_bwd_dst_f32")
            split, _scratch2 = g.bwd.split_arg(C + 1, dev)
            with _Timed("faconv_bwd_src"):
                _lib.check(lib.rgbx_faconv_bwd_src_f32(_lib.ptr(g.bwd.rowptr), _lib.ptr(g.bwd.col), _lib.ptr(g.w_t),
                                                       _lib.ptr(t2f), px, ldx, _lib.ptr(alr), pg, ldg, att[0].data_ptr(),
                                                       att[1].data_ptr(), _lib.ptr(g_alr), pgx, ldgx, N, C, _lib.ptr(seed),
                                                       p_drop, None if split is None else ctypes.byref(split),
                                                       _lib.stream_ptr()), "rgbx_faconv_bwd_src_f32")
        else:
            _, q = _faconv_edge_coef(g.fwd, g.w, None, alr, 0, seed, p_drop, True)
            _faconv_edge_dot(g.fwd, q, gout, x, g_alr, 1)
            coef_t, q_t = _faconv_edge_coef(g.bwd, g.w_t, t2f, alr, 1, seed, p_drop, True)
            _faconv_edge_dot(g.bwd, q_t, x, gout, g_alr, 0)
            g_x = torch.addmm(spmm_raw(g.bwd, coef_t, None, gout, kind="faconv_bwd_composed"), g_alr, att)
        g_att = gemm_tn(g_alr, x)
        g_x0 = gout * ctx.eps if ctx.use_x0 and ctx.needs_input_grad[1] else None
        return (g_x, g_x0, g_att[0].reshape(ctx.att_shapes[0]), g_att[1].reshape(ctx.att_shapes[1]), None, None, None,
                None, None, None)


def faconv(x, x0, att_l, att_r, graph, eps=0.1, training=False, p_drop=0.0, form=None, record=None):
    if _is_dist(graph):
        raise RuntimeError("FAConv has no node-partitioned form: run it on one GPU")
    _lib.require_device(x, x0, att_l, att_r)
    if not (0.0 <= p_drop < 1.0):
        raise ValueError("faconv: dropout must be in [0, 1)")
    return _FAConv.apply(x, x0, att_l, att_r, graph, float(eps), bool(training), float(p_drop),
                         faconv_form(x.size(1), form), record)


def _scores_in_kernel(C):
    vec = 4 if C % 4 == 0 else (2 if C % 2 == 0 else 1)
    lanes = 1
    while lanes * vec < C:
        lanes *= 2
    return lanes <= 8


def gather_rows(src, idx, out=None):
    _lib.require_device(src, idx)
    ps, lds = _lib.mat(src, "src")
    n, d = idx.numel(), src.size(1)
    if out is None:
        out = torch.empty((n, d), dtype=torch.float32, device=src.device)
    po, ldo = _lib.mat(out, "dst")
    _lib.check(_lib.load().rgbx_gather_rows_f32(ps, lds, _lib.ptr(idx), n, d, po, ldo, _lib.stream_ptr()),
               "rgbx_gather_rows_f32")
    return out


def scatter_add_rows(src, idx, dst):
    _lib.require_device(src, idx, dst)
    ps, lds = _lib.mat(src, "src")
    pd, ldd = _lib.mat(dst, "dst")
    _lib.check(
        _lib.load().rgbx_scatter_add_rows_f32(ps, lds, _lib.ptr(idx), idx.numel(), src.size(1), pd, ldd,
                                              _lib.stream_ptr()), "rgbx_scatter_add_rows_f32")
    return dst



def gemm_tn(a, b, alpha=1.0, colsum=False, out=None, sums_out=None):
    _lib.require_device(a, b)
    a = a if a.stride(-1) == 1 and _rows_padded_readable(a) else a.contiguous()
    b = b if b.stride(-1) == 1 and _rows_padded_readable(b) else b.contiguous()
    if a.size(0) >= 4096:
        a, b = (_aligned_rows(t) for t in (a, b))
    pa, lda = _lib.mat(a, "a")
    pb, ldb = _lib.mat(b, "b")
    K, M, N = a.size(0), a.size(1), b.size(1)
    lib = _lib.load()
    nbytes = ctypes.c_size_t(0)
    _lib.check(lib.rgbx_gemm_tn_workspace_bytes(K, M, N, ctypes.byref(nbytes)), "rgbx_gemm_tn_workspace_bytes")
    ws = torch.empty(max(nbytes.value, 1), dtype=torch.uint8, device=a.device)
    if out is None:
        out = torch.empty((M, N), dtype=torch.float32, device=a.device)
    elif tuple(out.shape) != (M, N) or not out.is_contiguous() or out.dtype != torch.float32:
        raise RuntimeError(f"gemm_tn: out must be a contiguous float32 [{M}, {N}] tensor")
    sums = None
    if colsum:
        sums = sums_out if sums_out is not None else torch.empty(M, dtype=torch.float32, device=a.device)
        if tuple(sums.shape) != (M,) or not sums.is_contiguous() or sums.dtype != torch.float32:
            raise RuntimeError(f"gemm_tn: sums_out must be a contiguous float32 [{M}] tensor")
    with _Timed("gemm_tn", f"{M}x{N}" if _EVENT_SINK is not None else None):
        _lib.check(lib.rgbx_gemm_tn_f32(pa, lda, pb, ldb, _lib.ptr(out), N, _lib.ptr(sums), K, M, N, float(alpha),
                                        _lib.ptr(ws), ws.numel(), _lib.stream_ptr()), "rgbx_gemm_tn_f32")
    return (out, sums) if colsum else out


class _Linear(torch.autograd.Function):

    @staticmethod
    def forward(ctx, x, weight, bias):
        ctx.save_for_backward(x, weight)
        ctx.has_bias = bias is not None
        if _EVENT_SINK is None or not x.is_cuda:
            return torch.nn.functional.linear(x, weight, bias)
        with _Timed("linear_fwd", f"{weight.size(1)}->{weight.size(0)}"):
            return torch.nn.functional.linear(x, weight, bias)

    @staticmethod
    def backward(ctx, gy):
        x, weight = ctx.saved_tensors
        gy = gy.contiguous()
        gx = gy @ weight if ctx.needs_input_grad[0] else None
        gw = gb = None
        want_b = ctx.has_bias and ctx.needs_input_grad[2]
        if ctx.needs_input_grad[1] and gy.is_cuda and want_b:
            gw, gb = gemm_tn(gy, x, colsum=True)
        else:
            if ctx.needs_input_grad[1]:
                gw = gemm_tn(gy, x) if gy.is_cuda else gy.t() @ x
            gb = gy.sum(0) if want_b else None
        return gx, gw, gb


def linear(x, weight, bias=None):
    sp = getattr(x, "_rgbx_sparse", None)
    if sp is not None and not x.requires_grad:
        return _SparseRowsLinear.apply(sp, weight, bias)
    return _Linear.apply(x, weight, bias)


SHORT_ROWS_TABLE_BYTES = 2 << 20
SHORT_ROWS_MEAN_SLOTS = 64


def short_rows_ok(csr, table):
    d = table.size(1)
    return (table.is_cuda and d % 4 == 0 and 4 <= d <= 64 and table.numel() * 4 <= SHORT_ROWS_TABLE_BYTES
            and csr.nnz <= SHORT_ROWS_MEAN_SLOTS * max(csr.N, 1))


def spmm_short_rows_raw(csr, w, x, bias=None, kind="spmm"):
    _lib.require_device(x, w, bias)
    px, ldx = _lib.mat(x, "x")
    N, d = csr.N, x.size(1)
    out = torch.empty((N, d), dtype=torch.float32, device=x.device)
    with _Timed(kind, f"shortrows+d{d}" if _EVENT_SINK is not None else None):
        _lib.check(_lib.load().rgbx_spmm_csr_short_rows_f32(_lib.ptr(csr.rowptr), _lib.ptr(csr.col), _lib.ptr(w), px, ldx,
                                                            _lib.ptr(bias), _lib.ptr(out), d, N, d, _lib.stream_ptr()),
                   "rgbx_spmm_csr_short_rows_f32")
    return out


class SparseFeatures:
    requires_grad = False

    def __init__(self, sp, like):
        self._rgbx_sparse, self.shape, self.device, self.dtype, self.is_cuda = sp, like.shape, like.device, like.dtype, True

    def size(self, dim=None):
        return self.shape if dim is None else self.shape[dim]

    def dim(self):
        return len(self.shape)


def dropout(x, p, training):
    sp = getattr(x, "_rgbx_sparse", None)
    if sp is None or not training or p <= 0.0 or x.requires_grad:
        return torch.nn.functional.dropout(x, p=p, training=training)
    if p >= 1.0:
        return SparseFeatures(sp.with_values(torch.zeros_like(sp.val)), x)
    keep = torch.rand(sp.val.numel(), device=sp.val.device) >= p
    return SparseFeatures(sp.with_values(sp.val * keep * (1.0 / (1.0 - p))), x)


class SparseRows:

    def __init__(self, x):
        from .graph import CSR, make_row_split
        _lib.require_device(x)
        n, f = x.shape
        step = max(1, (1 << 28) // max(f, 1))
        rows, cols, vals = [], [], []
        for r0 in range(0, n, step):
            blk = x[r0:r0 + step]
            nz = blk.nonzero(as_tuple=False)
            rows.append(nz[:, 0] + r0)
            cols.append(nz[:, 1].contiguous())
            vals.append(blk[nz[:, 0], nz[:, 1]])
        rows, cols, vals = (torch.cat(t).contiguous() if t else x.new_zeros(0, dtype=dt)
                            for t, dt in ((rows, torch.int64), (cols, torch.int64), (vals, x.dtype)))
        self.n, self.f, self.nnz = n, f, int(rows.numel())
        if self.nnz >= 2 ** 31 - 1:
            raise RuntimeError("SparseRows: more than 2^31 non-zeros")
        i32 = lambda t: t.to(torch.int32).contiguous()

        def rowptr_of(idx, m):
            ptr = torch.zeros(m + 1, dtype=torch.int64, device=x.device)
            ptr[1:] = torch.cumsum(torch.bincount(idx, minlength=m), 0)
            return i32(ptr)

        pad = lambda t: t if t.numel() else t.new_zeros(1)
        ptr = rowptr_of(rows, n)
        self.fwd = CSR(ptr, pad(i32(cols)), None, n, self.nnz, make_row_split(ptr))
        self.val = pad(vals)
        order = torch.argsort(cols, stable=True)
        self.order = order
        ptr_t = rowptr_of(cols, f)
        self.bwd = CSR(ptr_t, pad(i32(rows[order])), None, f, self.nnz, make_row_split(ptr_t))
        self.val_t = pad(vals[order].contiguous())

    def with_values(self, vals):
        import copy
        other = copy.copy(self)
        other.val = vals.contiguous()
        other.val_t = vals[self.order].contiguous() if self.nnz else vals
        return other


class _SparseRowsLinear(torch.autograd.Function):

    @staticmethod
    def forward(ctx, sp, weight, bias):
        ctx.sp, ctx.has_bias = sp, bias is not None
        wt = weight.detach().t().contiguous()
        b = None if bias is None else bias.detach().contiguous()
        if short_rows_ok(sp.fwd, wt):
            return spmm_short_rows_raw(sp.fwd, sp.val, wt, bias=b, kind="features_fwd")
        return spmm_raw(sp.fwd, sp.val, None, wt, kind="features_fwd", bias=b)

    @staticmethod
    def backward(ctx, gy):
        sp = ctx.sp
        gy = gy.contiguous()
        gw = gb = None
        if ctx.needs_input_grad[1]:
            gw = spmm_raw(sp.bwd, sp.val_t, None, gy, kind="features_bwd").t()
        if ctx.has_bias and ctx.needs_input_grad[2]:
            gb = gy.sum(0)
        return None, gw, gb


def prepare_features(x, max_density=0.1):
    x = align_rows(x)
    if x.dim() == 2 and x.is_cuda and x.dtype == torch.float32 and not x.requires_grad and x.numel():
        step = max(1, (1 << 28) // x.size(1))
# ... 137 lines not shown
```

Before: 17.07 billion.

## Add row-list and fused BN-backward forms to gemm_tn for dense tail

Measured after the change: 17.56 billion (median of 6 runs). 2.9% higher.

```diff
diff --git a/include/rgbx_hip.h b/include/rgbx_hip.h
--- a/include/rgbx_hip.h
+++ b/include/rgbx_hip.h
@@ -313,6 +313,22 @@
                      float* a_colsum, int64_t K, int64_t M, int64_t N, float alpha, void* workspace,
                      size_t workspace_bytes, rgbx_stream_t stream);
 
+typedef struct rgbx_gemm_tn_t {
+  const float* A; int64_t lda;
+  const float* B; int64_t ldb;
+  float* C; int64_t ldc;
+  float* a_colsum;
+  int64_t K, M, N;
+  float alpha;
+  void* workspace; size_t workspace_bytes;
+  int32_t row_list;
+  const int32_t* rows; int64_t n_rows;
+  const float* x; int64_t ldx;
+  const float *mean, *rstd, *ca, *cb, *ck;
+} rgbx_gemm_tn_t;
+
+int rgbx_gemm_tn_ex_f32(const rgbx_gemm_tn_t* g, rgbx_stream_t stream);
+
 
 int rgbx_bn_scratch_doubles(int64_t N, int64_t d, int64_t* count);
 
diff --git a/rgb_experiment_amd/_lib.py b/rgb_experiment_amd/_lib.py
--- a/rgb_experiment_amd/_lib.py
+++ b/rgb_experiment_amd/_lib.py
@@ -37,6 +37,13 @@
                 ("pre_scale", _P), ("pre_shift", _P), ("pre_rowsum", _P), ("out_colsums", _P), ("stats_ws", _P),
                 ("stats_ws_bytes", ctypes.c_size_t), ("ce", _P), ("N", _I64), ("K", _I64), ("Nout", _I64),
                 ("split", _P), ("w_pos", _P), ("z_pos_out", _P), ("col_sel", _P)]
+
+
+class GemmTn(ctypes.Structure):
+    _fields_ = [("A", _P), ("lda", _I64), ("B", _P), ("ldb", _I64), ("C", _P), ("ldc", _I64), ("a_colsum", _P),
+                ("K", _I64), ("M", _I64), ("N", _I64), ("alpha", _F), ("workspace", _P),
+                ("workspace_bytes", ctypes.c_size_t), ("row_list", ctypes.c_int32), ("rows", _P), ("n_rows", _I64),
+                ("x", _P), ("ldx", _I64), ("mean", _P), ("rstd", _P), ("ca", _P), ("cb", _P), ("ck", _P)]
 
 
 SIGNATURES = {
@@ -107,6 +114,7 @@
     "rgbx_gatv2_draws_u8": [_P, _I64, _I, _F, _P, _P],
     "rgbx_gemm_tn_workspace_bytes": [_I64, _I64, _I64, ctypes.POINTER(ctypes.c_size_t)],
     "rgbx_gemm_tn_f32": [_P, _I64, _P, _I64, _P, _I64, _P, _I64, _I64, _I64, _F, _P, ctypes.c_size_t, _P],
+    "rgbx_gemm_tn_ex_f32": [_P, _P],
     "rgbx_bn_scratch_doubles": [_I64, _I64, ctypes.POINTER(ctypes.c_int64)],
     "rgbx_bn_stats_f32": [_P, _I64, _I64, _I64, _P, _P, _I64, _P],
     "rgbx_bn_finalize_f32": [_P, _P, _P, _F, _F, _P, _P, _P, _P, _P, _P, _I64, _P],
diff --git a/rgb_experiment_amd/csrc/bn.hip b/rgb_experiment_amd/csrc/bn.hip
--- a/rgb_experiment_amd/csrc/bn.hip
+++ b/rgb_experiment_amd/csrc/bn.hip
@@ -147,7 +147,7 @@
     load_vec<VEC>(b, cb + c);
     load_vec<VEC>(k, ck + c);
 #pragma unroll
-    for (int i = 0; i < VEC; ++i) g[i] = (g[i] - a[i] - (v[i] - mu[i]) * rs[i] * b[i]) * k[i];
+    for (int i = 0; i < VEC; ++i) g[i] = bn_bwd_map(g[i], v[i], mu[i], rs[i], a[i], b[i], k[i]);
     store_vec<VEC>(gx + r * ldgx + c, g);
   }
 }
diff --git a/rgb_experiment_amd/csrc/gemm.hip b/rgb_experiment_amd/csrc/gemm.hip
--- a/rgb_experiment_amd/csrc/gemm.hip
+++ b/rgb_experiment_amd/csrc/gemm.hip
@@ -42,12 +42,68 @@
   }
 }
 
+template <int MT>
+struct WaveTile {
+  static constexpr int MI = MT / 64;
+  f32x16 acc[MI][2];
+  float csum;
+  int wm, wn, kr, cc;
+
+  __device__ __forceinline__ void init() {
+    const int wave = threadIdx.x >> 6, lane = threadIdx.x & 63;
+    wm = (wave >> 1) * (MT / 2), wn = (wave & 1) * 64;
+    kr = lane >> 5, cc = lane & 31;
+    csum = 0.f;
+#pragma unroll
+    for (int i = 0; i < MI; ++i)
+#pragma unroll
+      for (int j = 0; j < 2; ++j)
+#pragma unroll
+        for (int r = 0; r < 16; ++r) acc[i][j][r] = 0.f;
+  }
+
+  __device__ __forceinline__ void consume(const float* __restrict__ la, const float* __restrict__ lb, bool sums) {
+    if (sums) {
+#pragma unroll 8
+      for (int r = 0; r < KT; ++r) csum += la[r * MT + threadIdx.x];
+    }
+#pragma unroll 4
+    for (int kk = 0; kk < KT; kk += 2) {
+      float a[MI];
+#pragma unroll
+      for (int i = 0; i < MI; ++i) a[i] = la[(kk + kr) * MT + wm + i * 32 + cc];
+      const float b0 = lb[(kk + kr) * 128 + wn + cc];
+      const float b1 = lb[(kk + kr) * 128 + wn + 32 + cc];
+#pragma unroll
+      for (int i = 0; i < MI; ++i) {
+        acc[i][0] = __builtin_amdgcn_mfma_f32_32x32x2f32(a[i], b0, acc[i][0], 0, 0, 0);
+        acc[i][1] = __builtin_amdgcn_mfma_f32_32x32x2f32(a[i], b1, acc[i][1], 0, 0, 0);
+      }
+    }
+  }
+
+  __device__ __forceinline__ void store(float* __restrict__ part, float* __restrict__ colpart, bool sums, int split,
+                                        int m0, int n0, int M, int N) const {
+    if (sums && m0 + (int)threadIdx.x < M) colpart[(int64_t)split * M + m0 + threadIdx.x] = csum;
+    float* out = part + (int64_t)split * M * N;
+#pragma unroll
+    for (int i = 0; i < MI; ++i)
+#pragma unroll
+      for (int j = 0; j < 2; ++j)
+#pragma unroll
+        for (int r = 0; r < 16; ++r) {
+          const int m = m0 + wm + i * 32 + (r & 3) + 8 * (r >> 2) + 4 * kr;
+          const int n = n0 + wn + j * 32 + cc;
+          if (m < M && n < N) out[(int64_t)m * N + n] = acc[i][j][r];
+        }
+  }
+};
+
 template <bool VEC4, int MT>
 __global__ void __launch_bounds__(256)
 gemm_tn_partial_kernel(const float* __restrict__ A, int64_t lda, const float* __restrict__ B, int64_t ldb,
                        float* __restrict__ part, float* __restrict__ colpart, int64_t K, int M, int N,
                        int64_t slab) {
-  constexpr int MI = MT / 64;
   __shared__ float lds[KT * (MT + 128)];
   float* la = lds;
   float* lb = lds + KT * MT;
@@ -55,39 +111,9 @@
   const int m0 = blockIdx.y * MT, n0 = blockIdx.z * BN;
   const int64_t k_begin = (int64_t)split * slab;
   const int64_t k_end = k_begin + slab < K ? k_begin + slab : K;
-  const int wave = threadIdx.x >> 6, lane = threadIdx.x & 63;
-  const int wm = (wave >> 1) * (MT / 2), wn = (wave & 1) * 64;
-  const int kr = lane >> 5, cc = lane & 31;
-
-  f32x16 acc[MI][2];
-#pragma unroll
-  for (int i = 0; i < MI; ++i)
-#pragma unroll
-    for (int j = 0; j < 2; ++j)
-#pragma unroll
-      for (int r = 0; r < 16; ++r) acc[i][j][r] = 0.f;
-
+  WaveTile<MT> T;
+  T.init();
   const bool sums = colpart != nullptr && blockIdx.z == 0 && threadIdx.x < MT;
-  float csum = 0.f;
-  auto consume = [&]() {
-    if (sums) {
-#pragma unroll 8
-      for (int r = 0; r < KT; ++r) csum += la[r * MT + threadIdx.x];
-    }
-#pragma unroll 4
-    for (int kk = 0; kk < KT; kk += 2) {
-      float a[MI];
-#pragma unroll
-      for (int i = 0; i < MI; ++i) a[i] = la[(kk + kr) * MT + wm + i * 32 + cc];
-      const float b0 = lb[(kk + kr) * 128 + wn + cc];
-      const float b1 = lb[(kk + kr) * 128 + wn + 32 + cc];
-#pragma unroll
-      for (int i = 0; i < MI; ++i) {
-        acc[i][0] = __builtin_amdgcn_mfma_f32_32x32x2f32(a[i], b0, acc[i][0], 0, 0, 0);
-        acc[i][1] = __builtin_amdgcn_mfma_f32_32x32x2f32(a[i], b1, acc[i][1], 0, 0, 0);
-      }
-    }
-  };
   if constexpr (VEC4) {
     float4 ra[KT * (MT / 4) / 256], rb[KT * 32 / 256];
     fetch_tile<MT>(ra, A, lda, k_begin, k_end, m0, M);
@@ -101,7 +127,7 @@
         fetch_tile<MT>(ra, A, lda, k0 + KT, k_end, m0, M);
         fetch_tile<128>(rb, B, ldb, k0 + KT, k_end, n0, N);
       }
-      consume();
+      T.consume(la, lb, sums);
     }
   } else {
     for (int64_t k0 = k_begin; k0 < k_end; k0 += KT) {
@@ -109,22 +135,154 @@
       stage_tile<MT>(la, A, lda, k0, k_end, m0, M);
       stage_tile<128>(lb, B, ldb, k0, k_end, n0, N);
       __syncthreads();
-      consume();
-    }
-  }
-
-  if (sums && m0 + (int)threadIdx.x < M) colpart[(int64_t)split * M + m0 + threadIdx.x] = csum;
-  float* out = part + (int64_t)split * M * N;
-#pragma unroll
-  for (int i = 0; i < MI; ++i)
-#pragma unroll
-    for (int j = 0; j < 2; ++j)
-#pragma unroll
-      for (int r = 0; r < 16; ++r) {
-        const int m = m0 + wm + i * 32 + (r & 3) + 8 * (r >> 2) + 4 * kr;
-        const int n = n0 + wn + j * 32 + cc;
-        if (m < M && n < N) out[(int64_t)m * N + n] = acc[i][j][r];
+      T.consume(la, lb, sums);
+    }
+  }
+  T.store(part, colpart, sums, split, m0, n0, M, N);
+}
+
+
+__device__ __forceinline__ int lower_bound_i32(const int32_t* __restrict__ rows, int n, int64_t key) {
+  int lo = 0, hi = n;
+  while (lo < hi) {
+    const int mid = (lo + hi) >> 1;
+    if ((int64_t)rows[mid] < key) lo = mid + 1; else hi = mid;
+  }
+  return lo;
+}
+
+template <int W>
+__device__ __forceinline__ void load_ids(int (&ids)[KT * (W / 4) / 256], const int32_t* __restrict__ rows, int64_t t0,
+                                         int64_t t_end, int64_t k_begin, int64_t k_end) {
+#pragma unroll
+  for (int p = 0; p < KT * (W / 4) / 256; ++p) {
+    const int r = (p * 256 + (int)threadIdx.x) / (W / 4);
+    int id = -1;
+    if (t0 + r < t_end) {
+      id = rows[t0 + r];
+      if (id < k_begin || id >= k_end) id = -1;
+    }
+    ids[p] = id;
+  }
+}
+
+template <int W>
+__device__ __forceinline__ void fetch_listed(float4 (&regs)[KT * (W / 4) / 256], const float* __restrict__ src, int64_t ld,
+                                             const int (&ids)[KT * (W / 4) / 256], int c0, int ncols) {
+#pragma unroll
+  for (int p = 0; p < KT * (W / 4) / 256; ++p) {
+    const int c = ((p * 256 + (int)threadIdx.x) % (W / 4)) * 4;
+    regs[p] = make_float4(0.f, 0.f, 0.f, 0.f);
+    if (ids[p] >= 0 && c0 + c < ncols) regs[p] = *reinterpret_cast<const float4*>(src + (int64_t)ids[p] * ld + c0 + c);
+  }
+}
+
+template <int W>
+__device__ __forceinline__ void put_tile_bn(float* __restrict__ lds, const float4 (&regs)[KT * (W / 4) / 256],
+                                            const float4 (&rx)[KT * (W / 4) / 256], const float* __restrict__ coef,
+                                            int nvalid, int c0, int ncols) {
+  const int c = ((int)threadIdx.x % (W / 4)) * 4;
+  const int rlim = c0 + c < ncols ? nvalid : 0;
+#pragma unroll
+  for (int h = 0; h < 2; ++h) {
+    const float2 mu = *reinterpret_cast<const float2*>(coef + 0 * W + c + 2 * h);
+    const float2 rs = *reinterpret_cast<const float2*>(coef + 1 * W + c + 2 * h);
+    const float2 ca = *reinterpret_cast<const float2*>(coef + 2 * W + c + 2 * h);
+    const float2 cb = *reinterpret_cast<const float2*>(coef + 3 * W + c + 2 * h);
+    const float2 ck = *reinterpret_cast<const float2*>(coef + 4 * W + c + 2 * h);
+#pragma unroll
+    for (int p = 0; p < KT * (W / 4) / 256; ++p) {
+      const int r = (p * 256 + (int)threadIdx.x) / (W / 4);
+      float2 g = h == 0 ? make_float2(regs[p].x, regs[p].y) : make_float2(regs[p].z, regs[p].w);
+      if (r < rlim) {
+        const float2 x = h == 0 ? make_float2(rx[p].x, rx[p].y) : make_float2(rx[p].z, rx[p].w);
+        g.x = bn_bwd_map(g.x, x.x, mu.x, rs.x, ca.x, cb.x, ck.x);
+        g.y = bn_bwd_map(g.y, x.y, mu.y, rs.y, ca.y, cb.y, ck.y);
       }
+      *reinterpret_cast<float2*>(lds + r * W + c + 2 * h) = g;
+    }
+    __builtin_amdgcn_sched_barrier(0);
+  }
+}
+
+struct BnMapArgs {
+  const float* x;
+  int64_t ldx;
+  const float *mean, *rstd, *ca, *cb, *ck;
+};
+
+template <int MT, bool ROWS, bool BNMAP>
+__global__ void __launch_bounds__(256) __attribute__((amdgpu_waves_per_eu(MT == 64 ? 4 : 3)))
+gemm_tn_forms_kernel(const float* __restrict__ A, int64_t lda, const float* __restrict__ B, int64_t ldb,
+                     float* __restrict__ part, float* __restrict__ colpart, int64_t K, int M, int N, int64_t slab,
+                     const int32_t* __restrict__ rows, int n_rows, BnMapArgs bn) {
+  constexpr int NA = KT * (MT / 4) / 256, NB = KT * 32 / 256;
+  __shared__ float lds[KT * (MT + 128) + (BNMAP ? 5 * MT : 0)];
+  float* la = lds;
+  float* lb = lds + KT * MT;
+  float* coef = lds + KT * (MT + 128);
+  const int split = blockIdx.x;
+  const int m0 = blockIdx.y * MT, n0 = blockIdx.z * BN;
+  const int64_t k_begin = (int64_t)split * slab;
+  const int64_t k_end = k_begin + slab < K ? k_begin + slab : K;
+  int64_t t_begin = k_begin, t_end = k_end;
+  if constexpr (ROWS) {
+    t_begin = lower_bound_i32(rows, n_rows, k_begin);
+    t_end = lower_bound_i32(rows, n_rows, k_end);
+  }
+  WaveTile<MT> T;
+  T.init();
+  const bool sums = colpart != nullptr && blockIdx.z == 0 && threadIdx.x < MT;
+  if constexpr (BNMAP) {
+    if (threadIdx.x < MT) {
+      const int c = m0 + threadIdx.x;
+      const bool ok = c < M;
+      coef[0 * MT + threadIdx.x] = ok ? bn.mean[c] : 0.f;
+      coef[1 * MT + threadIdx.x] = ok ? bn.rstd[c] : 0.f;
+      coef[2 * MT + threadIdx.x] = ok ? bn.ca[c] : 0.f;
+      coef[3 * MT + threadIdx.x] = ok ? bn.cb[c] : 0.f;
+      coef[4 * MT + threadIdx.x] = ok ? bn.ck[c] : 0.f;
+    }
+  }
+  float4 ra[NA], rb[NB], rx[BNMAP ? NA : 1];
+  int ia[ROWS ? NA : 1], ib[ROWS ? NB : 1];
+  auto fetch = [&](int64_t t0) {
+    if constexpr (ROWS) {
+      fetch_listed<MT>(ra, A, lda, ia, m0, M);
+      if constexpr (BNMAP) fetch_listed<MT>(rx, bn.x, bn.ldx, ia, m0, M);
+      fetch_listed<128>(rb, B, ldb, ib, n0, N);
+    } else {
+      fetch_tile<MT>(ra, A, lda, t0, t_end, m0, M);
+      if constexpr (BNMAP) fetch_tile<MT>(rx, bn.x, bn.ldx, t0, t_end, m0, M);
+      fetch_tile<128>(rb, B, ldb, t0, t_end, n0, N);
+    }
+  };
+  auto ids = [&](int64_t t0) {
+    if constexpr (ROWS) {
+      load_ids<MT>(ia, rows, t0, t_end, k_begin, k_end);
+      load_ids<128>(ib, rows, t0, t_end, k_begin, k_end);
+    }
+  };
+  ids(t_begin);
+  fetch(t_begin);
+  ids(t_begin + KT);
+  for (int64_t t0 = t_begin; t0 < t_end; t0 += KT) {
+    __syncthreads();
+    put_tile<128>(lb, rb);
+    if constexpr (BNMAP) {
+      const int64_t left = t_end - t0;
+      put_tile_bn<MT>(la, ra, rx, coef, left < KT ? (int)left : KT, m0, M);
+    } else {
+      put_tile<MT>(la, ra);
+    }
+    __syncthreads();
+    if (t0 + KT < t_end) {
+      fetch(t0 + KT);
+      ids(t0 + 2 * KT);
+    }
+    T.consume(la, lb, sums);
+  }
+  T.store(part, colpart, sums, split, m0, n0, M, N);
 }
 
 __global__ void __launch_bounds__(256)
@@ -209,3 +367,64 @@
   }
   return RGBX_OK;
 }
+
+extern "C" int rgbx_gemm_tn_ex_f32(const rgbx_gemm_tn_t* g, rgbx_stream_t stream) {
+  if (!g) return fail(RGBX_E_ARG, "gemm_tn_ex: null descriptor");
+  const bool listed = g->row_list != 0;
+  const bool mapped = g->x != nullptr;
+  if (!listed && !mapped)
+    return rgbx_gemm_tn_f32(g->A, g->lda, g->B, g->ldb, g->C, g->ldc, g->a_colsum, g->K, g->M, g->N, g->alpha,
+                            g->workspace, g->workspace_bytes, stream);
+  if (listed && mapped) return fail(RGBX_E_ARG, "gemm_tn_ex: a row list and the map cannot be combined in one call");
+  const int64_t K = g->K, M = g->M, N = g->N;
+  if (K < 0 || M < 0 || N < 0 || g->n_rows < 0) return fail(RGBX_E_ARG, "gemm_tn_ex: negative size");
+  if (M == 0 || N == 0) return RGBX_OK;
+  if (!g->C || (K > 0 && (!g->A || !g->B))) return fail(RGBX_E_ARG, "gemm_tn_ex: null pointer");
+  if (M >= INT32_MAX || N >= INT32_MAX) return fail(RGBX_E_RANGE, "gemm_tn_ex: M or N exceeds int32");
+  if (g->lda < M || g->ldb < N || g->ldc < N) return fail(RGBX_E_ARG, "gemm_tn_ex: leading dimension too small");
+  if (listed) {
+    if (g->n_rows > 0 && !g->rows) return fail(RGBX_E_ARG, "gemm_tn_ex: n_rows > 0 without a row list");
+    if (K >= INT32_MAX || g->n_rows > K) return fail(RGBX_E_RANGE, "gemm_tn_ex: a row list needs n_rows <= K < 2^31");
+  }
+  if (!(aligned16(g->A) && aligned16(g->B) && g->lda % 4 == 0 && g->ldb % 4 == 0))
+    return fail(RGBX_E_ALIGN, "gemm_tn_ex: operand forms need 16-byte aligned rows of A and B");
+  if (mapped) {
+    if (!g->mean || !g->rstd || !g->ca || !g->cb || !g->ck) return fail(RGBX_E_ARG, "gemm_tn_ex: x without its coefficients");
+    if (M % 4 != 0 || g->ldx < M || g->ldx % 4 != 0 || !aligned16(g->x))
+      return fail(RGBX_E_ALIGN, "gemm_tn_ex: the map needs M %% 4 == 0 and 16-byte aligned rows of x");
+  }
+  size_t need = 0;
+  if (int rc = rgbx_gemm_tn_workspace_bytes(K, M, N, &need)) return rc;
+  if (!g->workspace || g->workspace_bytes < need)
+    return fail(RGBX_E_WS, "gemm_tn_ex: workspace %zu < %zu bytes", g->workspace_bytes, need);
+  hipStream_t s = (hipStream_t)stream;
+  const int S = choose_splits(K, (int)M, (int)N);
+  const int64_t slab = cdiv(cdiv(K > 0 ? K : 1, S), KT) * KT;
+  float* part = static_cast<float*>(g->workspace);
+  float* colpart = g->a_colsum ? part + (size_t)S * M * N : nullptr;
+  const int mt = tile_rows((int)M);
+  dim3 grid(S, (unsigned)cdiv(M, mt), (unsigned)cdiv(N, BN));
+  const BnMapArgs bn{g->x, g->ldx, g->mean, g->rstd, g->ca, g->cb, g->ck};
+#define RGBX_GEMM_TN_FORM(MT, RL, BN_)                                                                                \
+  gemm_tn_forms_kernel<MT, RL, BN_><<<grid, 256, 0, s>>>(g->A, g->lda, g->B, g->ldb, part, colpart, K, (int)M, (int)N, \
+                                                      slab, g->rows, (int)g->n_rows, bn)
+  if (mt == 64) {
+    if (listed) RGBX_GEMM_TN_FORM(64, true, false);
+    else RGBX_GEMM_TN_FORM(64, false, true);
+  } else {
+    if (listed) RGBX_GEMM_TN_FORM(128, true, false);
+    else RGBX_GEMM_TN_FORM(128, false, true);
+  }
+#undef RGBX_GEMM_TN_FORM
+  RGBX_CHECK_LAUNCH("gemm_tn_forms_kernel");
+  const int64_t MN = M * N;
+  int64_t rb = cdiv(MN, 32);
+  if (rb > kMaxGrid) rb = kMaxGrid;
+  gemm_tn_reduce_kernel<<<(int)rb, 256, 0, s>>>(part, S, MN, g->C, (int)N, g->ldc, g->alpha);
+  RGBX_CHECK_LAUNCH("gemm_tn_reduce_kernel");
+  if (g->a_colsum) {
+    gemm_tn_reduce_kernel<<<(int)cdiv(M, 32), 256, 0, s>>>(colpart, S, M, g->a_colsum, (int)M, M, 1.0f);
+    RGBX_CHECK_LAUNCH("gemm_tn_reduce_kernel");
+  }
+  return RGBX_OK;
+}
diff --git a/rgb_experiment_amd/csrc/rgbx_common.h b/rgb_experiment_amd/csrc/rgbx_common.h
--- a/rgb_experiment_amd/csrc/rgbx_common.h
+++ b/rgb_experiment_amd/csrc/rgbx_common.h
@@ -69,6 +69,12 @@
   *reinterpret_cast<V*>(p) = t;
 }
 
+__device__ __forceinline__ float bn_bwd_map(float g, float x, float mean, float rstd, float ca, float cb, float ck) {
+#pragma clang fp contract(off)
+  const float xhat = (x - mean) * rstd;
+  return fmaf(-xhat, cb, g - ca) * ck;
+}
+
 constexpr int kMaxGrid = 256 * 8 * 4;
 
 }
diff --git a/rgb_experiment_amd/models/_stack.py b/rgb_experiment_amd/models/_stack.py
--- a/rgb_experiment_amd/models/_stack.py
+++ b/rgb_experiment_amd/models/_stack.py
@@ -97,6 +97,7 @@
             ew["edge_weight"] = edge_weight
         learned = edge_weight is not None and edge_weight.requires_grad and torch.is_grad_enabled()
         pending = None
+        handover = None
         if self.training and torch.is_grad_enabled():
             self._train_forwards = getattr(self, "_train_forwards", 0) + 1
         folded = self._eval_operands() if (not torch.is_grad_enabled() and not self.training and x.is_cuda) else None
@@ -129,6 +130,14 @@
             if (i == last and ce is not None and getattr(conv, "accepts_ce", False)
                     and (not isinstance(ce[1], (tuple, list)) or getattr(conv, "accepts_ce_pair", False))):
                 extra["ce"] = ce
+            if (i == 0 and bn is not None and bn.training and torch.is_grad_enabled() and x.is_cuda and not x.requires_grad
+                    and not learned and getattr(conv, "accepts_bn_backward", False) and hasattr(bn, "begin_training_step")
+                    and getattr(self.convs[1], "accepts_bn_backward", False) and ops.dense_tail_fusion()
+                    and not _any_module_hooks(conv, bn, self.convs[1])):
+                handover = ops.BNHandover()
+                extra["bn_handover"] = handover
+            elif i == 1 and handover is not None and handover.armed and pending is not None:
+                extra["bn_handover"] = handover
             if pending is not None:
                 sums = getattr(x, ops.COLSUMS, None)
                 after = getattr(conv, "forward_after_bn", None)
@@ -147,6 +156,14 @@
         if ce is not None and not isinstance(x, tuple):
             x = ops.ce_from_logits(x, ce[0], ce[1])
         return x
+
+
+def _any_module_hooks(*modules):
+    import torch.nn.modules.module as M
+    tables = ("_forward_hooks", "_forward_pre_hooks", "_backward_hooks", "_backward_pre_hooks")
+    glob = ("_global_forward_hooks", "_global_forward_pre_hooks", "_global_backward_hooks", "_global_backward_pre_hooks")
+    present = lambda owner, name: not hasattr(owner, name) or bool(getattr(owner, name))
+    return any(present(m, t) for m in modules for t in tables) or any(present(M, t) for t in glob)
 
 
 def _layer_maps(conv):
diff --git a/rgb_experiment_amd/nn/batchnorm.py b/rgb_experiment_amd/nn/batchnorm.py
--- a/rgb_experiment_amd/nn/batchnorm.py
+++ b/rgb_experiment_amd/nn/batchnorm.py
@@ -113,7 +113,7 @@
     return mean, rstd, scale, shift, n
 
 
-def train_backward(gy, x, weight, mean, rstd, n, reduce, grads_out=None, sums=None):
+def train_backward(gy, x, weight, mean, rstd, n, reduce, grads_out=None, sums=None, apply=True):
     gy = gy if gy.stride(-1) == 1 else gy.contiguous()
     d = x.size(1)
     if sums is None:
@@ -139,6 +139,8 @@
             grads_out[0].copy_(gw)
             grads_out[1].copy_(gb)
             gw, gb = grads_out
+    if not apply:
+        return (ca, cb, ck), gw, gb
     return bwd_apply(gy, x, mean, rstd, ca, cb, ck), gw, gb
 
 
diff --git a/rgb_experiment_amd/nn/conv.py b/rgb_experiment_amd/nn/conv.py
--- a/rgb_experiment_amd/nn/conv.py
+++ b/rgb_experiment_amd/nn/conv.py
@@ -103,15 +103,16 @@
 
     accepts_ce = True
     accepts_ce_pair = True
-
-    def forward(self, x, edge_index, edge_weight=None, post_affine=None, want_colsums=False, ce=None):
+    accepts_bn_backward = True
+
+    def forward(self, x, edge_index, edge_weight=None, post_affine=None, want_colsums=False, ce=None, bn_handover=None):
         if ce is not None:
             return self._ce(x, edge_index, ce, None, None, edge_weight)
         weight, bias = self.lin.weight, self.bias
         if post_affine is not None:
             scale, shift = post_affine
             weight, bias = weight * scale[:, None], bias * scale + shift
-        return self._conv(x, edge_index, weight, bias, want_colsums, edge_weight)
+        return self._conv(x, edge_index, weight, bias, want_colsums, edge_weight, bn_handover)
 
     def eval_operands(self, bn=None):
         return ops.fold_bn_linear(self.lin.weight, self.bias, bn=bn)
@@ -133,7 +134,7 @@
     def _learned(edge_weight):
         return edge_weight is not None and edge_weight.requires_grad and torch.is_grad_enabled()
 
-    def _ce(self, x, edge_index, ce, bn, colsums, edge_weight=None):
+    def _ce(self, x, edge_index, ce, bn, colsums, edge_weight=None, bn_handover=None):
         y, mask = ce
         if self._learned(edge_weight):
             if bn is not None:
@@ -143,7 +144,7 @@
         hand_over = bn is not None and bn.folds_into_next_layer(x)
         if ops.fused_ce_ok(graph, self.in_channels, self.out_channels, False, x, y) and (bn is None or hand_over):
             return ops.propagate_linear_ce(x, graph, "gcn", self.lin.weight, self.bias, None, y, mask, bn=bn,
-                                           colsums=colsums)
+                                           colsums=colsums, handover=bn_handover)
         if bn is not None:
             x = bn(x, colsums=colsums)
         weight, bias, n = ops.pad_rows4(self.lin.weight, self.bias)
@@ -151,24 +152,25 @@
             return ops.propagate_rows_ce(ops.linear(x, weight), graph, "gcn", n, self.out_channels, y, mask, bias=bias)
         return ops.ce_from_logits(self.forward(x, edge_index, edge_weight), y, mask)
 
-    def forward_after_bn(self, x, edge_index, bn, colsums=None, want_colsums=False, ce=None, edge_weight=None):
+    def forward_after_bn(self, x, edge_index, bn, colsums=None, want_colsums=False, ce=None, edge_weight=None,
+                         bn_handover=None):
         if ce is not None:
-            return self._ce(x, edge_index, ce, bn, colsums, edge_weight)
+            return self._ce(x, edge_index, ce, bn, colsums, edge_weight, bn_handover)
         if self._learned(edge_weight):
             return self.forward(bn(x, colsums=colsums), edge_index, edge_weight, want_colsums=want_colsums)
         graph = get_graph(edge_index, x.size(0), LOOPS_ADD_REMAINING, edge_weight)
         if (bn.folds_into_next_layer(x) and not getattr(graph, "is_distributed", False)
                 and ops.fused_linear_ok(graph, self.in_channels, self.out_channels, x=x)):
             return ops.bn_propagate_linear(x, bn, graph, "gcn", self.lin.weight, self.bias, colsums=colsums,
-                                           want_colsums=want_colsums)
+                                           want_colsums=want_colsums, handover=bn_handover)
         return self.forward(bn(x, colsums=colsums), edge_index, edge_weight, want_colsums=want_colsums)
 
-    def _conv(self, x, edge_index, weight, bias, want_colsums=False, edge_weight=None):
+    def _conv(self, x, edge_index, weight, bias, want_colsums=False, edge_weight=None, bn_handover=None):
         graph = get_graph(edge_index, x.size(0), LOOPS_ADD_REMAINING, edge_weight)
         if self._learned(edge_weight):
             return ops.propagate_gcn_edge_weight(ops.linear(x, weight), edge_weight, graph, bias=bias)
         if ops.fused_linear_ok(graph, self.in_channels, self.out_channels, x=x):
-            return ops.propagate_linear(x, graph, "gcn", weight, bias, want_colsums=want_colsums)
+            return ops.propagate_linear(x, graph, "gcn", weight, bias, want_colsums=want_colsums, handover=bn_handover)
         if not x.requires_grad and self.in_channels <= self.out_channels:
             return ops.linear(ops.propagate_gcn(x, graph), weight, bias)
         if want_colsums and ops.rows_epilogue_ok(graph, self.out_channels, x):
diff --git a/rgb_experiment_amd/ops.py b/rgb_experiment_amd/ops.py
--- a/rgb_experiment_amd/ops.py
+++ b/rgb_experiment_amd/ops.py
@@ -773,10 +773,35 @@
     return wt, b_out, wrt
 
 
+class BNHandover:
+    __slots__ = ("armed", "grad", "map")
+
+    def __init__(self):
+        self.armed, self.grad, self.map = False, None, None
+
+    def leave(self, g_h, bn_map):
+        self.grad, self.map = g_h, bn_map
+
+    def take(self, gy):
+        g, m = self.grad, self.map
+        self.grad = self.map = None
+        if m is None:
+            return None
+        if g is not gy and (g.data_ptr() != gy.data_ptr() or tuple(g.shape) != tuple(gy.shape)):
+            raise RuntimeError("BatchNorm backward hand-over: the first conv received a gradient other than the one the "
+                               "BatchNorm's node left for it (ops.set_dense_tail_fusion(False) runs the separate pass)")
+        return m
+
+
 class _PropagateLinear(torch.autograd.Function):
 
     @staticmethod
-    def forward(ctx, x, graph, kind, weight, bias, need_z=True, root_weight=None, x_root=None, want_colsums=False):
+    def forward(ctx, x, graph, kind, weight, bias, need_z=True, root_weight=None, x_root=None, want_colsums=False,
+                handover=None):
+        ctx.handover = None
+        if handover is not None and root_weight is None and not x.requires_grad and need_z:
+            handover.armed = True
+            ctx.handover = handover
         x = x.contiguous()
         xr = x if x_root is None else x_root.contiguous()
         w = graph.w if kind == "gcn" else None
@@ -799,12 +824,17 @@
     def backward(ctx, gy, _g_colsums=None):
         z, weight, root_weight, x = ctx.saved_tensors
         g, kind = ctx.graph, ctx.kind
+        bn_map = ctx.handover.take(gy) if ctx.handover is not None else None
+        if bn_map is not None and (not ctx.needs_input_grad[3] or ctx.needs_input_grad[0]):
+            from .nn import batchnorm as B
+            gy, bn_map = B.bwd_apply(gy.contiguous(), *bn_map), None
         gy = gy.contiguous()
         gx = gw = gb = gwr = None
         want_b = ctx.has_bias and ctx.needs_input_grad[4]
         if ctx.needs_input_grad[3]:
-            if want_b:
-                gw, gb = gemm_tn(gy, z, colsum=True)
+            if want_b or bn_map is not None:
+                gw, gb = gemm_tn(gy, z, colsum=True, bn_map=bn_map)
+                gb = gb if want_b else None
             else:
                 gw = gemm_tn(gy, z)
         elif want_b:
@@ -813,7 +843,7 @@
             gwr = gemm_tn(gy, x)
         if ctx.needs_input_grad[0]:
             gx = _propagate_linear_input_grad(g, kind, gy, weight, root_weight)
-        return gx, None, None, gw, gb, None, gwr, None, None
+        return gx, None, None, gw, gb, None, gwr, None, None, None
 
 
 def _propagate_linear_input_grad(g, kind, gy, weight, root_weight, ce_sel=None):
@@ -838,8 +868,9 @@
 
     @staticmethod
     def forward(ctx, x, bn_weight, bn_bias, graph, kind, weight, bias, root_weight, eps, reduce, running, need_z,
-                colsums=None, want_colsums=False):
+                colsums=None, want_colsums=False, handover=None):
         from .nn import batchnorm as B
+        ctx.handover = handover if handover is not None and handover.armed and x.is_contiguous() else None
         x = x.contiguous()
         mean, rstd, scale, shift, n = B.train_statistics(x, bn_weight, bn_bias, eps, reduce, running, colsums)
         w, rs = (graph.w, None) if kind == "gcn" else (None, graph.inv_deg)
@@ -871,8 +902,18 @@
         if root_weight is not None and ctx.needs_input_grad[7]:
             gwr = gemm_tn(gy, x) * scale + gcol[:, None] * shift
         g_h = _propagate_linear_input_grad(g, kind, gy, weight, root_weight)
-        gx, g_bnw, g_bnb = B.train_backward(g_h, x, bn_weight, mean, rstd, n, ctx.reduce)
-        return gx, g_bnw, g_bnb, None, None, gw, gb, gwr, None, None, None, None, None, None
+        gx, g_bnw, g_bnb = _bn_backward(ctx.handover, g_h, x, bn_weight, mean, rstd, n, ctx.reduce)
+        return gx, g_bnw, g_bnb, None, None, gw, gb, gwr, None, None, None, None, None, None, None
+
+
+def _bn_backward(handover, g_h, x, bn_weight, mean, rstd, n, reduce):
+    from .nn import batchnorm as B
+    if handover is None:
+        return B.train_backward(g_h, x, bn_weight, mean, rstd, n, reduce)
+    g_h = g_h if g_h.is_contiguous() else g_h.contiguous()
+    coefs, g_bnw, g_bnb = B.train_backward(g_h, x, bn_weight, mean, rstd, n, reduce, apply=False)
+    handover.leave(g_h, (x, mean, rstd) + tuple(coefs))
+    return g_h, g_bnw, g_bnb
 
 
 _SCALE_CACHE = {}
@@ -939,7 +980,6 @@
 
 _SEL_COLS = {}
 
-
 def selected_cols(y, mask, C):
     key = _sel_key(y, mask, C)
     hit = _SEL_COLS.get(key)
@@ -971,8 +1011,12 @@
 class _PropagateLinearCE(torch.autograd.Function):
 
     @staticmethod
-    def forward(ctx, x, graph, kind, weight, bias, root_weight, y, mask, want_grad, bn_weight, bn_bias, bn_args):
+    def forward(ctx, x, graph, kind, weight, bias, root_weight, y, mask, want_grad, bn_weight, bn_bias, bn_args,
+                handover=None):
         from .nn import batchnorm as B
+        ctx.handover = (handover if handover is not None and handover.armed and bn_weight is not None
+                        and x.is_contiguous() else None)
+        ctx.rows_form = dense_tail_fusion()
         x = x.contiguous()
         pre = None
         if bn_weight is not None:
@@ -1011,16 +1055,17 @@
         g = g.reshape(()).float()
         gw = gb = gwr = gx = g_bnw = g_bnb = None
         gcol = None
+        rows = selected_rows(*ctx.ce_sel) if ctx.rows_form and ctx.ce_sel is not None else None
         if ctx.needs_input_grad[3]:
-            gw, gcol = gemm_tn(gy, z, colsum=True)
+            gw, gcol = gemm_tn(gy, z, colsum=True, rows=rows)
         if ctx.has_bias and ctx.needs_input_grad[4]:
             gb = gcol if gcol is not None else gy.sum(0)
         if root_weight is not None and ctx.needs_input_grad[5]:
             if ctx.has_bn:
                 gcol = gcol if gcol is not None else gy.sum(0)
-                gwr = gemm_tn(gy, x) * scale + gcol[:, None] * shift
+                gwr = gemm_tn(gy, x, rows=rows) * scale + gcol[:, None] * shift
             else:
-                gwr = gemm_tn(gy, x)
+                gwr = gemm_tn(gy, x, rows=rows)
         need_h = ctx.needs_input_grad[0] or (ctx.has_bn and (ctx.needs_input_grad[9] or ctx.needs_input_grad[10]))
         items = [(k, t) for k, t in (("gw", gw), ("gb", gb), ("gwr", gwr)) if t is not None]
         if need_h:
@@ -1032,27 +1077,29 @@
         if need_h:
             g_h = _propagate_linear_input_grad(graph, kind, gy, sc["w"], sc.get("wr"), ce_sel=ctx.ce_sel)
             if ctx.has_bn:
-                gx, g_bnw, g_bnb = B.train_backward(g_h, x, bn_weight, mean, rstd, n, ctx.reduce)
+                gx, g_bnw, g_bnb = _bn_backward(ctx.handover, g_h, x, bn_weight, mean, rstd, n, ctx.reduce)
             else:
                 gx = g_h
-        return gx, None, None, gw, gb, gwr, None, None, None, g_bnw, g_bnb, None
-
-
-def propagate_linear_ce(x, graph, kind, weight, bias, root_weight, y, mask, bn=None, colsums=None):
+        return gx, None, None, gw, gb, gwr, None, None, None, g_bnw, g_bnb, None, None
+
+
+def propagate_linear_ce(x, graph, kind, weight, bias, root_weight, y, mask, bn=None, colsums=None, handover=None):
     want_grad = not isinstance(mask, (tuple, list)) and torch.is_grad_enabled() and any(
         t is not None and t.requires_grad
         for t in (weight, x, bias, root_weight) + ((bn.weight, bn.bias) if bn is not None else ()))
     if bn is not None:
         bn_args = (bn.eps, bn._reduce, bn.begin_training_step(), colsums)
         return _PropagateLinearCE.apply(x, graph, kind, weight, bias, root_weight, y, mask, want_grad, bn.weight, bn.bias,
-                                        bn_args)
+                                        bn_args, handover)
     return _PropagateLinearCE.apply(x, graph, kind, weight, bias, root_weight, y, mask, want_grad, None, None, None)
 
 
-def bn_propagate_linear(x, bn, graph, kind, weight, bias=None, root_weight=None, colsums=None, want_colsums=False):
+def bn_propagate_linear(x, bn, graph, kind, weight, bias=None, root_weight=None, colsums=None, want_colsums=False,
+                        handover=None):
     need_z = weight.requires_grad
     return _tag_colsums(_BNPropagateLinear.apply(x, bn.weight, bn.bias, graph, kind, weight, bias, root_weight, bn.eps,
-                                                 bn._reduce, bn.begin_training_step(), need_z, colsums, want_colsums),
+                                                 bn._reduce, bn.begin_training_step(), need_z, colsums, want_colsums,
+                                                 handover),
                         want_colsums)
 
 
@@ -1067,11 +1114,12 @@
     return out
 
 
-def propagate_linear(x, graph, kind, weight, bias=None, root_weight=None, want_colsums=False):
+def propagate_linear(x, graph, kind, weight, bias=None, root_weight=None, want_colsums=False, handover=None):
     if _is_dist(graph):
         return graph.propagate_linear(x, kind, weight, bias, root_weight)
     need_z = torch.is_grad_enabled() and weight.requires_grad
-    return _tag_colsums(_PropagateLinear.apply(x, graph, kind, weight, bias, need_z, root_weight, None, want_colsums),
+    return _tag_colsums(_PropagateLinear.apply(x, graph, kind, weight, bias, need_z, root_weight, None, want_colsums,
+                                               handover),
                         want_colsums)
 
 
@@ -2158,12 +2206,49 @@
 
 
 
-def gemm_tn(a, b, alpha=1.0, colsum=False, out=None, sums_out=None):
-    _lib.require_device(a, b)
+_DENSE_TAIL_FUSION = [True]
+
+
+def set_dense_tail_fusion(on):
+    prev = _DENSE_TAIL_FUSION[0]
+    _DENSE_TAIL_FUSION[0] = bool(on)
+    return prev
+
+
+def dense_tail_fusion():
+    return _DENSE_TAIL_FUSION[0]
+
+
+def _vec_rows(t):
+    return t.stride(-1) == 1 and t.stride(0) % 4 == 0 and t.data_ptr() % 16 == 0
+
+
+def gemm_tn(a, b, alpha=1.0, colsum=False, out=None, sums_out=None, rows=None, bn_map=None, check_rows=False):
+    _lib.require_device(a, b, rows)
+    if rows is not None:
+        if rows.device != a.device:
+            raise RuntimeError(f"gemm_tn: rows are on {rows.device}, the matrices on {a.device}")
+        if check_rows and rows.numel():
+            r = rows.long()
+            if not bool(((r[1:] > r[:-1]).all() & (r[0] >= 0) & (r[-1] < a.size(0))).item()):
+                raise RuntimeError("gemm_tn: rows must be ascending, distinct and inside [0, K)")
+    if bn_map is not None:
+        x = bn_map[0]
+        x = x if x.stride(-1) == 1 else x.contiguous()
+        fits = (rows is None and a.size(1) % 4 == 0 and tuple(x.shape) == tuple(a.shape) and _vec_rows(a) and _vec_rows(b)
+                and _vec_rows(x) and all(v.is_contiguous() and v.dtype == torch.float32 for v in bn_map[1:]))
+        if not fits:
+            from .nn import batchnorm as B
+            return gemm_tn(B.bwd_apply(a.contiguous(), x, *bn_map[1:]), b, alpha, colsum, out, sums_out, rows=rows)
+        bn_map = (x,) + tuple(bn_map[1:])
     a = a if a.stride(-1) == 1 and _rows_padded_readable(a) else a.contiguous()
     b = b if b.stride(-1) == 1 and _rows_padded_readable(b) else b.contiguous()
     if a.size(0) >= 4096:
         a, b = (_aligned_rows(t) for t in (a, b))
+    if rows is not None and not (_vec_rows(a) and _vec_rows(b)):
+        rows = None
+    if rows is not None and (rows.dtype != torch.int32 or rows.dim() != 1 or not rows.is_contiguous()):
+        raise RuntimeError(f"gemm_tn: rows must be a contiguous int32 vector, got {rows.dtype} {tuple(rows.shape)}")
     pa, lda = _lib.mat(a, "a")
     pb, ldb = _lib.mat(b, "b")
     K, M, N = a.size(0), a.size(1), b.size(1)
@@ -2180,9 +2265,24 @@
         sums = sums_out if sums_out is not None else torch.empty(M, dtype=torch.float32, device=a.device)
         if tuple(sums.shape) != (M,) or not sums.is_contiguous() or sums.dtype != torch.float32:
             raise RuntimeError(f"gemm_tn: sums_out must be a contiguous float32 [{M}] tensor")
-    with _Timed("gemm_tn", f"{M}x{N}" if _EVENT_SINK is not None else None):
-        _lib.check(lib.rgbx_gemm_tn_f32(pa, lda, pb, ldb, _lib.ptr(out), N, _lib.ptr(sums), K, M, N, float(alpha),
-                                        _lib.ptr(ws), ws.numel(), _lib.stream_ptr()), "rgbx_gemm_tn_f32")
+    if rows is None and bn_map is None:
+        with _Timed("gemm_tn", f"{M}x{N}" if _EVENT_SINK is not None else None):
+            _lib.check(lib.rgbx_gemm_tn_f32(pa, lda, pb, ldb, _lib.ptr(out), N, _lib.ptr(sums), K, M, N, float(alpha),
+                                            _lib.ptr(ws), ws.numel(), _lib.stream_ptr()), "rgbx_gemm_tn_f32")
+        return (out, sums) if colsum else out
+    G = _lib.GemmTn(A=pa, lda=lda, B=pb, ldb=ldb, C=_lib.ptr(out), ldc=N, a_colsum=_lib.ptr(sums), K=K, M=M, N=N,
+                    alpha=float(alpha), workspace=_lib.ptr(ws), workspace_bytes=ws.numel())
+    form = []
+    if rows is not None:
+        G.row_list, G.rows, G.n_rows = 1, _lib.ptr(rows), rows.numel()
+        form.append("rows")
+    if bn_map is not None:
+        x, mean, rstd, ca, cb, ck = bn_map
+        G.x, G.ldx = _lib.mat(x, "x")
+        G.mean, G.rstd, G.ca, G.cb, G.ck = (_lib.ptr(v) for v in (mean, rstd, ca, cb, ck))
+        form.append("bn")
+    with _Timed("gemm_tn", f"{M}x{N}+{'+'.join(form)}" if _EVENT_SINK is not None else None):
+        _lib.check(lib.rgbx_gemm_tn_ex_f32(ctypes.byref(G), _lib.stream_ptr()), "rgbx_gemm_tn_ex_f32")
     return (out, sums) if colsum else out
 
 
```
